# salemmohammed/Distributed-TensorFlow-Guide

Measured on AMD Instinct MI355X. Metric: images/sec (whole node) ResNet-50 sync DP at 1/2/4/8 MI355X; scaling efficiency, higher is better.
Workload: dtype bf16; 1 GPU; model=ResNet-50, global_batch=1024, per_gpu_batch=1024, image_size=224, optimizer=momentum-sgd (fused), parallelism=dp1, allreduce=rccl bf16, 8 MB buckets, overlapped, step_launch=eager

## Files before the change

csrc/bindings/ops.cc:

```cpp
#include <torch/extension.h>
#include <c10/core/DeviceGuard.h>
#include <c10/hip/HIPStream.h>

#include "dtg/kernels.h"

namespace {

using at::Tensor;
using dtg::bf16_t;

hipStream_t cur_stream() { return c10::hip::getCurrentHIPStream().stream(); }

at::Tensor zeros_f32(long long n, const at::Tensor& like) {
  c10::DeviceGuard dg(like.device());
  at::Tensor t = at::empty({n}, like.options().dtype(at::kFloat));
  dtg::fill_zero(t.data_ptr(), n * 4, cur_stream());
  return t;
}

#define CHECK_CUDA(x) TORCH_CHECK((x).is_cuda(), #x " must be a GPU tensor")
#define CHECK_CONTIG(x) TORCH_CHECK((x).is_contiguous(), #x " must be contiguous")
#define CHECK_DT(x, dt) TORCH_CHECK((x).scalar_type() == (dt), #x " must be " #dt)
#define CHECK_IN(x) \
  CHECK_CUDA(x);    \
// ... 707 lines not shown
    CHECK_DT(*bias, at::kFloat);
    TORCH_CHECK(bias->numel() == N, "bias size mismatch");
    bptr = bias->data_ptr<float>();
  }
  void* auxp = nullptr;
  if (aux_mode != 0) {
    TORCH_CHECK(aux_mode >= 1 && aux_mode <= 4, "aux_mode in {0, 1, 2, 3, 4}");
    TORCH_CHECK(aux_mode != 3 || act != 0, "aux_mode 3 stores act'(pre): needs an activation");
    TORCH_CHECK(aux.has_value() && aux->defined(), "aux_mode needs an aux tensor");
    TORCH_CHECK(aux->is_cuda() && aux->scalar_type() == at::kBFloat16 && aux->dim() == 2, "aux must be bf16 2-D");
    TORCH_CHECK(aux->size(0) == M && aux->size(1) == N && aux->stride(0) == out.stride(0) && aux->stride(1) == 1,
                "aux must match out's shape and row stride");
    auxp = aux->data_ptr();
  }
  c10::DeviceGuard dg(A.device());
  if (colsum.has_value() && colsum->defined()) {
    CHECK_IN(*colsum);
    CHECK_DT(*colsum, at::kFloat);
    TORCH_CHECK(colsum->numel() == N, "colsum must hold N floats");
    TORCH_CHECK(a_kc && !b_kc && out.scalar_type() == at::kBFloat16 && alpha == 1.0 && beta == 0.0,
                "colsum epilogue: A [M,K], B [K,N], bf16 out, alpha 1, beta 0");
    TORCH_CHECK(out.stride(0) % 8 == 0 && N % 8 == 0 && ((uintptr_t)out.data_ptr() % 16) == 0 &&
                    (bptr == nullptr || ((uintptr_t)bptr % 16) == 0) && (auxp == nullptr || ((uintptr_t)auxp % 16) == 0),
                "colsum epilogue needs 16-byte aligned rows");
    dtg::gemm_bf16_colsum(cbfp(A), A.stride(0), cbfp(B), B.stride(0), bfp(out), out.stride(0), M, N, K, bptr, (int)act,
                          auxp, (int)aux_mode, colsum->data_ptr<float>(), cur_stream());
    return;
  }
  int sk = split_k > 0 ? (int)split_k : dtg::gemm_pick_split(M, N, K, a_kc ? 1 : 0);
  Tensor ws;
  float* wsp = nullptr;
  if (sk > 1) {
    ws = at::empty({dtg::gemm_workspace_floats(M, N, K, sk)}, A.options().dtype(at::kFloat));
    wsp = ws.data_ptr<float>();
  }
  dtg::gemm_bf16(cbfp(A), A.stride(0), a_kc, cbfp(B), B.stride(0), b_kc, out.data_ptr(), out.stride(0),
                 out.scalar_type() == at::kBFloat16, M, N, K, (float)alpha, (float)beta, bptr, (int)act, sk, wsp,
                 cur_stream(), dtg::GemmBatch(), auxp, (int)aux_mode);
}

void check_nhwc(const Tensor& t, const char* what) {
  CHECK_CUDA(t);
  TORCH_CHECK(t.scalar_type() == at::kBFloat16, what, " must be bf16");
  TORCH_CHECK(t.dim() == 4 && t.is_contiguous(), what, " must be a contiguous [N,H,W,C] tensor");
  TORCH_CHECK(((uintptr_t)t.data_ptr() % 16) == 0, what, " must be 16-byte aligned");
}

bool conv_supported(int64_t C, int64_t K, int64_t R, int64_t S, int64_t stride, int64_t pad, int64_t which) {
  return dtg::conv_supported((int)C, (int)K, (int)R, (int)S, (int)stride, (int)pad, (int)which) != 0;
}

Tensor conv_fwd(Tensor x, Tensor w, int64_t stride, int64_t pad) {
  check_nhwc(x, "x");
  check_nhwc(w, "w");
  const int N = x.size(0), H = x.size(1), W = x.size(2), C = x.size(3);
  const int K = w.size(0), R = w.size(1), S = w.size(2);
  TORCH_CHECK(w.size(3) == C, "weight channels mismatch");
  TORCH_CHECK(dtg::conv_supported(C, K, R, S, stride, pad, 0), "conv shape not supported by the HIP kernel");
  const int P = (H + 2 * pad - R) / stride + 1, Q = (W + 2 * pad - S) / stride + 1;
  TORCH_CHECK(P > 0 && Q > 0, "empty output");
  TORCH_CHECK((long long)N * H * W * C < (1LL << 31) && (long long)N * P * Q * K < (1LL << 31), "tensor too large");
  c10::DeviceGuard dg(x.device());
  auto y = at::empty({N, P, Q, K}, x.options());
  dtg::conv_fwd(cbfp(x), cbfp(w), bfp(y), N, H, W, C, K, R, S, stride, pad, cur_stream());
  return y;
}


Tensor conv_dgrad(Tensor dy, Tensor w, int64_t H, int64_t W, int64_t stride, int64_t pad, c10::optional<Tensor> out,
                  double beta, bool zero_rest) {
  check_nhwc(dy, "dy");
  check_nhwc(w, "w");
  const int N = dy.size(0), P = dy.size(1), Q = dy.size(2), K = dy.size(3);
  const int R = w.size(1), S = w.size(2), C = w.size(3);
  TORCH_CHECK(w.size(0) == K, "weight/dy channel mismatch");
  TORCH_CHECK(dtg::conv_supported(C, K, R, S, stride, pad, 1), "dgrad shape not supported by the HIP kernel");
  TORCH_CHECK((H + 2 * pad - R) / stride + 1 == P && (W + 2 * pad - S) / stride + 1 == Q, "dgrad geometry mismatch");
  c10::DeviceGuard dg(dy.device());
  Tensor dx;
  if (out.has_value()) {
    dx = *out;
    check_nhwc(dx, "out");
    TORCH_CHECK(dx.size(0) == N && dx.size(1) == H && dx.size(2) == W && dx.size(3) == C, "out shape mismatch");
  } else {
    TORCH_CHECK(beta == 0.0, "beta != 0 needs out");
    dx = at::empty({N, H, W, C}, dy.options());
  }
  Tensor wT;
  TORCH_CHECK(zero_rest || (stride == 2 && R == 1 && S == 1 && pad == 0 && beta == 0.0),
              "zero_rest=False is for a stride-2 1x1 dgrad (beta 0)");
  dtg::conv_dgrad(cbfp(dy), cbfp(w), bfp(dx), N, H, W, C, K, R, S, stride, pad, (float)beta, cur_stream(),
                  dtg::BnEpi(), wT.defined() ? cbfp(wT) : nullptr, zero_rest ? 1 : 0);
  return dx;
}

std::tuple<Tensor, Tensor> conv_fwd_c8(Tensor x, Tensor w, int64_t R, int64_t S, int64_t stride, int64_t pad,
                                       bool with_stats, int64_t stride_w) {
  check_nhwc(x, "x");
  CHECK_IN(w);
  CHECK_DT(w, at::kBFloat16);
  const int sw = stride_w > 0 ? (int)stride_w : (int)stride;
  const int N = x.size(0), H = x.size(1), W = x.size(2), K = w.size(0);
  TORCH_CHECK(x.size(3) == 8, "conv_fwd_c8 needs 8 input channels");
  TORCH_CHECK(w.dim() == 2 && w.size(1) == (R * S * 8 + 63) / 64 * 64, "w must be [K, ceil64(R*S*8)]");
  TORCH_CHECK(K % 64 == 0, "K % 64");
  TORCH_CHECK(stride > 0 && sw > 0 && pad >= 0, "bad stride / pad");
  const int P = (H + 2 * pad - R) / stride + 1, Q = (W + 2 * pad - S) / sw + 1;
  TORCH_CHECK(P > 0 && Q > 0 && (long long)N * P * Q * K < (1LL << 31), "bad geometry");
  c10::DeviceGuard dg(x.device());
  auto y = at::empty({N, P, Q, K}, x.options());
  Tensor part;
  dtg::BnEpi bn;
  if (with_stats) {
    part = zeros_f32((long long)dtg::kBnStatSlots * 2 * K, x);
    bn.part = part.data_ptr<float>();
    bn.mode = 1;
  } else {
    part = at::empty({0}, x.options().dtype(at::kFloat));
  }
  dtg::conv_fwd_c8(cbfp(x), cbfp(w), bfp(y), N, H, W, K, (int)R, (int)S, (int)stride, (int)pad, cur_stream(), bn, sw);
  return {y, part};
}

constexpr int kPartRing = 16;
constexpr long long kPartCap = (long long)dtg::kBnStatSlots * 2 * 2048;
Tensor bn_part(const Tensor& like, int64_t C, bool pooled = false) {
  if (!pooled || C > 2048) return zeros_f32((long long)dtg::kBnStatSlots * 2 * C, like);
  static Tensor* ring = new Tensor[64];
  static int next[64] = {0};
  const int dev = like.get_device();
  TORCH_CHECK(dev >= 0 && dev < 64, "device index");
  if (!ring[dev].defined()) ring[dev] = zeros_f32((long long)kPartRing * kPartCap, like);
  const int i = next[dev]++ % kPartRing;
  return ring[dev].narrow(0, i * kPartCap, (long long)dtg::kBnStatSlots * 2 * C);
}

dtg::BnEpi bn_bwd_epi(Tensor& part, const Tensor& x, const Tensor& mean, const Tensor& invstd, const Tensor& gamma,
                      const Tensor& beta, long long M, int C) {
  CHECK_IN(x);
  CHECK_DT(x, at::kBFloat16);
  TORCH_CHECK(x.numel() == M * C, "BN input shape mismatch");
  for (const Tensor* t : {&mean, &invstd, &gamma, &beta}) {
    CHECK_IN(*t);
    CHECK_DT(*t, at::kFloat);
    TORCH_CHECK(t->numel() == C, "per-channel tensor size mismatch");
  }
  dtg::BnEpi bn;
  bn.part = part.data_ptr<float>();
  bn.mode = 2;
  bn.x = cbfp(x);
  bn.mean = mean.data_ptr<float>();
  bn.invstd = invstd.data_ptr<float>();
  bn.gamma = gamma.data_ptr<float>();
  bn.beta = beta.data_ptr<float>();
  return bn;
}

std::tuple<Tensor, Tensor> gemm_bn(Tensor A, Tensor B, int64_t mode, c10::optional<Tensor> x,
                                   c10::optional<Tensor> mean, c10::optional<Tensor> invstd,
                                   c10::optional<Tensor> gamma, c10::optional<Tensor> beta,
                                   c10::optional<Tensor> mask, c10::optional<Tensor> out, bool pooled,
                                   c10::optional<Tensor> x2, c10::optional<Tensor> mean2,
                                   c10::optional<Tensor> invstd2, c10::optional<Tensor> part2,
                                   c10::optional<std::tuple<int64_t, int64_t>> sub2_hw) {
  CHECK_IN(A);
  CHECK_DT(A, at::kBFloat16);
  CHECK_CUDA(B);
  CHECK_DT(B, at::kBFloat16);
  TORCH_CHECK(mode >= 1 && mode <= 3, "mode in {1, 2, 3}");
  TORCH_CHECK(A.dim() == 2 && B.dim() == 2 && B.stride(1) == 1, "2-D operands, contiguous rows");
  const int M = (int)A.size(0), K = (int)A.size(1);
  const int N = (int)(mode == 1 ? B.size(0) : B.size(1));
  TORCH_CHECK((mode == 1 ? B.size(1) : B.size(0)) == K, "gemm_bn K mismatch");
  TORCH_CHECK(K % 8 == 0 && N % 8 == 0 && B.stride(0) % 8 == 0, "K, N and row strides must be multiples of 8");
  TORCH_CHECK(((uintptr_t)A.data_ptr() % 16) == 0 && ((uintptr_t)B.data_ptr() % 16) == 0, "16-byte alignment");
  c10::DeviceGuard dg(A.device());
  Tensor o;
  float bt = 0.f;
  if (out.has_value() && out->defined()) {
    TORCH_CHECK(mode == 3, "accumulating into `out` is mode 3 only");
    o = *out;
    CHECK_IN(o);
    CHECK_DT(o, at::kBFloat16);
    TORCH_CHECK(o.numel() == (long long)M * N, "out shape mismatch");
    bt = 1.f;
  } else {
    o = at::empty({M, N}, A.options());
  }
  auto part = bn_part(A, N, pooled);
  dtg::BnEpi bn;
  if (mode >= 2) {
    TORCH_CHECK(x && mean && invstd && gamma && beta, "modes 2/3 need x, mean, invstd, gamma, beta");
    bn = bn_bwd_epi(part, *x, *mean, *invstd, *gamma, *beta, M, N);
    if (mode == 3) {
      TORCH_CHECK(mask.has_value() && mask->defined(), "mode 3 needs the mask tensor");
      CHECK_IN(*mask);
      bn.mode = 3;
      if (x2.has_value() && x2->defined()) {
        TORCH_CHECK(mean2 && invstd2 && part2, "x2 needs mean2, invstd2 and part2");
        CHECK_IN(*x2);
        CHECK_DT(*x2, at::kBFloat16);
        TORCH_CHECK(x2->numel() == (long long)M * N, "x2 shape mismatch");
        for (const Tensor* t : {&*mean2, &*invstd2}) {
          CHECK_IN(*t);
          CHECK_DT(*t, at::kFloat);
          TORCH_CHECK(t->numel() == N, "per-channel tensor size mismatch");
        }
        CHECK_IN(*part2);
        CHECK_DT(*part2, at::kFloat);
        TORCH_CHECK(part2->numel() == (long long)dtg::kBnStatSlots * 2 * N, "part2 size mismatch");
        bn.x2 = cbfp(*x2);
        bn.mean2 = mean2->data_ptr<float>();
        bn.invstd2 = invstd2->data_ptr<float>();
        bn.part2 = part2->data_ptr<float>();
      }
      if (sub2_hw.has_value()) {
        const auto [sh, sw] = *sub2_hw;
        TORCH_CHECK(bt != 0.f && sh > 0 && sw > 0 && (long long)M % (sh * sw) == 0, "sub2_hw needs out and M = N*H*W");
        dtg::bn_sub2_rows(bn, (int)sh, (int)sw);
      }
      if (mask->scalar_type() == at::kByte) {
        TORCH_CHECK(mask->numel() == (long long)M * (N / 8), "mask bits shape mismatch");
        bn.maskbits = mask->data_ptr<uint8_t>();
      } else {
        CHECK_DT(*mask, at::kBFloat16);
        TORCH_CHECK(mask->numel() == (long long)M * N, "mask shape mismatch");
        bn.mask = cbfp(*mask);
      }
    }
  } else {
    bn.part = part.data_ptr<float>();
    bn.mode = 1;
  }
  dtg::gemm_bf16_bn(cbfp(A), A.stride(0), cbfp(B), B.stride(0), bfp(o), N, M, N, K, bt, bn, cur_stream());
  return {o, part};
}

std::tuple<Tensor, Tensor> conv_fwd_bn(Tensor x, Tensor w, int64_t stride, int64_t pad, bool pooled) {
  check_nhwc(x, "x");
  check_nhwc(w, "w");
  const int N = x.size(0), H = x.size(1), W = x.size(2), C = x.size(3);
  const int K = w.size(0), R = w.size(1), S = w.size(2);
  TORCH_CHECK(w.size(3) == C, "weight channels mismatch");
  TORCH_CHECK(dtg::conv_supported(C, K, R, S, stride, pad, 0), "conv shape not supported by the HIP kernel");
  const int P = (H + 2 * pad - R) / stride + 1, Q = (W + 2 * pad - S) / stride + 1;
  TORCH_CHECK(P > 0 && Q > 0, "empty output");
  TORCH_CHECK((long long)N * H * W * C < (1LL << 31) && (long long)N * P * Q * K < (1LL << 31), "tensor too large");
  c10::DeviceGuard dg(x.device());
  auto y = at::empty({N, P, Q, K}, x.options());
  auto part = bn_part(x, K, pooled);
  dtg::BnEpi bn;
  bn.part = part.data_ptr<float>();
  bn.mode = 1;
  dtg::conv_fwd(cbfp(x), cbfp(w), bfp(y), N, H, W, C, K, R, S, stride, pad, cur_stream(), bn);
  return {y, part};
}

uint8_t* bits_ptr(const c10::optional<Tensor>& bits, long long M, int C) {
  if (!bits.has_value() || !bits->defined()) return nullptr;
  CHECK_IN(*bits);
  TORCH_CHECK(bits->scalar_type() == at::kByte && bits->numel() == M * (C / 8), "bits must be uint8 [M, C/8]");
  return bits->data_ptr<uint8_t>();
}

std::tuple<Tensor, Tensor> conv_dgrad_bn(Tensor dy, Tensor w, int64_t H, int64_t W, int64_t stride, int64_t pad,
                                         Tensor x, Tensor mean, Tensor invstd, Tensor gamma, Tensor beta,
                                         bool pooled, c10::optional<Tensor> bits) {
  check_nhwc(dy, "dy");
  check_nhwc(w, "w");
  const int N = dy.size(0), P = dy.size(1), Q = dy.size(2), K = dy.size(3);
  const int R = w.size(1), S = w.size(2), C = w.size(3);
  TORCH_CHECK(w.size(0) == K, "weight/dy channel mismatch");
  TORCH_CHECK(dtg::conv_supported(C, K, R, S, stride, pad, 1), "dgrad shape not supported by the HIP kernel");
  TORCH_CHECK((H + 2 * pad - R) / stride + 1 == P && (W + 2 * pad - S) / stride + 1 == Q, "dgrad geometry mismatch");
  c10::DeviceGuard dg(dy.device());
  auto dx = at::empty({N, H, W, C}, dy.options());
  auto part = bn_part(dy, C, pooled);
  dtg::BnEpi bn = bn_bwd_epi(part, x, mean, invstd, gamma, beta, (long long)N * H * W, C);
  if (uint8_t* mb = bits_ptr(bits, (long long)N * H * W, C)) {
    bn.mode = 3;
    bn.maskbits = mb;
  }
  Tensor wT;
  TORCH_CHECK(dtg::conv_dgrad(cbfp(dy), cbfp(w), bfp(dx), N, H, W, C, K, R, S, stride, pad, 0.f, cur_stream(), bn,
                              wT.defined() ? cbfp(wT) : nullptr),
              "conv_dgrad_bn: geometry leaves rows unwritten (use conv_dgrad + bn_bwd)");
  return {dx, part};
}

static void check_f32(std::initializer_list<const Tensor*> ts, long long n, const char* what) {
  for (const Tensor* t : ts) {
    CHECK_IN(*t);
    CHECK_DT(*t, at::kFloat);
    TORCH_CHECK(t->numel() == n, what, " size mismatch");
  }
}
static void check_per_channel(std::initializer_list<const Tensor*> ts, int C) {
  check_f32(ts, C, "per-channel tensor");
}
static void check_partials(std::initializer_list<const Tensor*> ts, int C) {
  check_f32(ts, (long long)dtg::kBnStatSlots * 2 * C, "partials");
}

std::tuple<Tensor, Tensor, Tensor> bn_fwd_part(Tensor x, Tensor part, c10::optional<Tensor> res, Tensor gamma,
                                               Tensor beta, Tensor rmean, Tensor rvar, double momentum, double eps,
                                               bool relu, c10::optional<Tensor> bits) {
  CHECK_IN(x);
  CHECK_DT(x, at::kBFloat16);
  TORCH_CHECK(x.dim() == 2, "x must be [M, C]");
  const long long M = x.size(0);
  const int C = (int)x.size(1);
  TORCH_CHECK(C % 8 == 0, "C must be a multiple of 8");
  check_partials({&part}, C);
  check_per_channel({&gamma, &beta, &rmean, &rvar}, C);
  const bool has_res = res.has_value() && res->defined();
  if (has_res) {
    CHECK_IN(*res);
    CHECK_DT(*res, at::kBFloat16);
    TORCH_CHECK(res->sizes() == x.sizes(), "residual shape mismatch");
  }
  c10::DeviceGuard dg(x.device());
  auto y = at::empty_like(x);
  auto fopt = x.options().dtype(at::kFloat);
  auto smean = at::empty({C}, fopt), sinv = at::empty({C}, fopt), ws = at::empty({2LL * C}, fopt);
  dtg::bn_fwd_from_part(cbfp(x), has_res ? cbfp(*res) : nullptr, bfp(y), gamma.data_ptr<float>(),
                        beta.data_ptr<float>(), rmean.data_ptr<float>(), rvar.data_ptr<float>(),
                        smean.data_ptr<float>(), sinv.data_ptr<float>(), part.data_ptr<float>(), ws.data_ptr<float>(),
                        M, C, (float)momentum, (float)eps, relu, cur_stream(), bits_ptr(bits, M, C));
  return {y, smean, sinv};
}

std::tuple<Tensor, Tensor, Tensor, Tensor, Tensor> bn_fwd2_part(Tensor x, Tensor part, Tensor gamma, Tensor beta,
                                                                Tensor rmean, Tensor rvar, Tensor r, Tensor part2,
                                                                Tensor gamma2, Tensor beta2, Tensor rmean2,
                                                                Tensor rvar2, double momentum, double eps,
                                                                c10::optional<Tensor> bits) {
  CHECK_IN(x);
  CHECK_IN(r);
  CHECK_DT(x, at::kBFloat16);
  CHECK_DT(r, at::kBFloat16);
  TORCH_CHECK(x.dim() == 2 && r.sizes() == x.sizes(), "x/r must be [M, C]");
  const long long M = x.size(0);
  const int C = (int)x.size(1);
  TORCH_CHECK(C % 8 == 0, "C must be a multiple of 8");
  check_partials({&part, &part2}, C);
  check_per_channel({&gamma, &beta, &rmean, &rvar, &gamma2, &beta2, &rmean2, &rvar2}, C);
  c10::DeviceGuard dg(x.device());
  auto y = at::empty_like(x);
  auto fopt = x.options().dtype(at::kFloat);
  auto m1 = at::empty({C}, fopt), i1 = at::empty({C}, fopt), m2 = at::empty({C}, fopt), i2 = at::empty({C}, fopt);
  auto ws = at::empty({4LL * C}, fopt);
  dtg::bn_fwd2_from_part(cbfp(x), cbfp(r), bfp(y), part.data_ptr<float>(), part2.data_ptr<float>(),
                         gamma.data_ptr<float>(), beta.data_ptr<float>(), rmean.data_ptr<float>(),
                         rvar.data_ptr<float>(), m1.data_ptr<float>(), i1.data_ptr<float>(), gamma2.data_ptr<float>(),
                         beta2.data_ptr<float>(), rmean2.data_ptr<float>(), rvar2.data_ptr<float>(),
                         m2.data_ptr<float>(), i2.data_ptr<float>(), ws.data_ptr<float>(), M, C, (float)momentum,
                         (float)eps, cur_stream(), bits_ptr(bits, M, C));
  return {y, m1, i1, m2, i2};
}

static void check_wgrad_fuse(const Tensor& x, const c10::optional<Tensor>& wact, const c10::optional<Tensor>& wgrad) {
  TORCH_CHECK(wact.has_value() && wgrad.has_value() && wact->defined() && wgrad->defined(), "wact needs wgrad");
  CHECK_CUDA(*wact);
  CHECK_DT(*wact, at::kBFloat16);
  CHECK_IN(*wgrad);
  TORCH_CHECK(wgrad->scalar_type() == at::kFloat || wgrad->scalar_type() == at::kBFloat16, "wgrad fp32/bf16");
  const long long M = x.size(0);
  const int C = (int)x.size(1), CI = (int)wact->size(1);
  TORCH_CHECK(wact->dim() == 2 && wact->size(0) == M && wact->stride(1) == 1 && wact->stride(0) % 8 == 0 &&
                  ((uintptr_t)wact->data_ptr() % 16) == 0,
              "wact must be [M, CI] with 16-byte aligned rows");
  TORCH_CHECK(wgrad->numel() == (long long)C * CI, "wgrad must be [C, CI]");
  TORCH_CHECK(dtg::bn_dx_wgrad_ok(M, C, CI), "fused dx + wgrad: unsupported shape (see bn_dx_wgrad_ok)");
}

struct DgradFuse {
  c10::optional<Tensor> w, y, mean, invstd, bits, part;
  bool full = false;
  bool on() const { return w.has_value() && w->defined(); }
};

static dtg::DxDgrad check_dgrad_fuse(const Tensor& x, const c10::optional<Tensor>& wact, const DgradFuse& f,
                                     const Tensor& dpo) {
  TORCH_CHECK(wact.has_value() && wact->defined(), "the fused dgrad rides on the fused weight gradient (wact)");
  for (const c10::optional<Tensor>* t : {&f.y, &f.mean, &f.invstd, &f.bits, &f.part})
    TORCH_CHECK(t->has_value() && (*t)->defined(), "dgw needs dgy, dgmean, dginv, dgbits and dgpart");
  const long long M = x.size(0);
  const int C = (int)x.size(1), CI = (int)wact->size(1);
  TORCH_CHECK(f.full || dtg::bn_dx_dgrad_ok(M, C, CI), "fused dx + dgrad: unsupported shape (see bn_dx_dgrad_ok)");
  TORCH_CHECK(!f.full || dtg::bn_dx_dgrad_full_ok(M, C, CI),
              "fused dx + dgrad: unsupported shape (see bn_dx_dgrad_full_ok)");
  CHECK_CUDA(*f.w);
  CHECK_DT(*f.w, at::kBFloat16);
  TORCH_CHECK(f.w->dim() == 2 && f.w->size(0) == C && f.w->size(1) == CI && f.w->stride(1) == 1 &&
                  f.w->stride(0) % 8 == 0 && ((uintptr_t)f.w->data_ptr() % 16) == 0,
              "dgw must be [C, CI] with 16-byte aligned rows");
  CHECK_IN(*f.y);
  CHECK_DT(*f.y, at::kBFloat16);
  TORCH_CHECK(f.y->dim() == 2 && f.y->size(0) == M && f.y->size(1) == CI && ((uintptr_t)f.y->data_ptr() % 16) == 0,
              "dgy must be [M, CI], 16-byte aligned");
  check_per_channel({&*f.mean, &*f.invstd}, CI);
  check_partials({&*f.part}, CI);
  dtg::DxDgrad d;
  d.w = cbfp(*f.w);
  d.ldw = f.w->stride(0);
  d.y = cbfp(*f.y);
  d.mean = f.mean->data_ptr<float>();
  d.invstd = f.invstd->data_ptr<float>();
  d.bits = bits_ptr(f.bits, M, CI);
  d.dp = bfp(dpo);
  d.part = f.part->data_ptr<float>();
  return d;
}

struct DxFuseSide {
  const Tensor &x, &part, &gamma, &smean, &sinv, &dgamma, &dbeta;
  const Tensor& dx;
  const c10::optional<Tensor> &wact, &wgrad;
};

static Tensor bn_dx_wgrad_fused(const Tensor& dp, const DxFuseSide& a, const DxFuseSide* b, const Tensor& ws, int accum,
                                const DgradFuse& dgf) {
  const long long M = a.x.size(0);
  const int C = (int)a.x.size(1);
  check_wgrad_fuse(a.x, a.wact, a.wgrad);
  const int CI = (int)a.wact->size(1);
  const bool w2 = b && b->wact.has_value() && b->wact->defined();
  if (w2) {
    check_wgrad_fuse(b->x, b->wact, b->wgrad);
    TORCH_CHECK(C == 256 && CI == 64 && b->wact->size(1) == CI && b->wgrad->scalar_type() == a.wgrad->scalar_type(),
                "wact2: 256 x 64 only, wgrad2 of wgrad's dtype");
  }
  Tensor dpo;
  dtg::DxDgrad dgd;
  if (dgf.on()) {
    TORCH_CHECK(!b || w2, "dgw in the dual form needs wact2");
    dpo = at::empty({M, (long long)CI}, a.x.options());
    dgd = check_dgrad_fuse(a.x, a.wact, dgf, dpo);
  }
  const long long ns = (long long)dtg::bn_dx_wgrad_slabs(C, CI, w2, dgf.on()) * C * CI;
  auto slabs = at::empty({w2 ? 2 * ns : ns}, a.x.options().dtype(at::kFloat));
  auto side = [&](const DxFuseSide& s, int k) {
    dtg::DxSide d;
    d.x = cbfp(s.x);
    float* coef = ws.data_ptr<float>() + k * 3LL * C;
    dtg::bn_bwd_coef_from_part(s.part.data_ptr<float>(), s.gamma.data_ptr<float>(), s.smean.data_ptr<float>(),
                               s.sinv.data_ptr<float>(), coef, s.dgamma.data_ptr<float>(), s.dbeta.data_ptr<float>(),
                               M, C, accum, cur_stream());
    d.coef = coef;
    d.dx = s.dx.defined() ? bfp(s.dx) : nullptr;
    if (s.wact.has_value() && s.wact->defined()) {
      d.act = cbfp(*s.wact);
      d.ldact = s.wact->stride(0);
      d.wgrad = s.wgrad->data_ptr();
      d.slabs = slabs.data_ptr<float>() + k * ns;
    }
    return d;
  };
  const dtg::DxSide da = side(a, 0), db = b ? side(*b, 1) : dtg::DxSide{};
  dtg::bn_dx_wgrad(cbfp(dp), da, b ? &db : nullptr, M, C, CI, a.wgrad->scalar_type() == at::kBFloat16, cur_stream(),
                   dgf.on() ? &dgd : nullptr);
  return dpo;
}

pybind11::tuple bn_bwd2_part(Tensor dp, Tensor x, Tensor part, Tensor gamma, Tensor smean, Tensor sinv,
                             Tensor dgamma, Tensor dbeta, Tensor x2, Tensor part2, Tensor gamma2,
                             Tensor smean2, Tensor sinv2, Tensor dgamma2, Tensor dbeta2,
                             c10::optional<Tensor> wact, c10::optional<Tensor> wgrad,
                             c10::optional<Tensor> wact2, c10::optional<Tensor> wgrad2,
                             c10::optional<Tensor> dgw, c10::optional<Tensor> dgy, c10::optional<Tensor> dgmean,
                             c10::optional<Tensor> dginv, c10::optional<Tensor> dgbits,
                             c10::optional<Tensor> dgpart, bool dgfull) {
  const DgradFuse dgf{dgw, dgy, dgmean, dginv, dgbits, dgpart, dgfull};
  TORCH_CHECK(!(dgfull && dgf.on()), "dgfull: the full-width fused dgrad has no dual form (bn_bwd_part only)");
  for (const Tensor* t : {&dp, &x, &x2}) {
    CHECK_IN(*t);
    CHECK_DT(*t, at::kBFloat16);
  }
  TORCH_CHECK(x.dim() == 2 && dp.numel() == x.numel() && x2.sizes() == x.sizes(), "dp/x/x2 must be [M, C]");
  const long long M = x.size(0);
  const int C = (int)x.size(1);
  TORCH_CHECK(C % 8 == 0, "C must be a multiple of 8");
  check_partials({&part, &part2}, C);
  check_per_channel({&gamma, &smean, &sinv, &dgamma, &dbeta, &gamma2, &smean2, &sinv2, &dgamma2, &dbeta2}, C);
  c10::DeviceGuard dg(x.device());
  TORCH_CHECK(!dgf.on() || (wact.has_value() && wact->defined()), "dgw needs wact");
  Tensor dx, dx2 = at::empty_like(x);
  if (!dgf.on()) dx = at::empty_like(x);
  auto ws = at::empty({6LL * C}, x.options().dtype(at::kFloat));
  if (wact.has_value() && wact->defined()) {
    const DxFuseSide a{x, part, gamma, smean, sinv, dgamma, dbeta, dx, wact, wgrad};
    const DxFuseSide b{x2, part2, gamma2, smean2, sinv2, dgamma2, dbeta2, dx2, wact2, wgrad2};
    const Tensor dpo = bn_dx_wgrad_fused(dp, a, &b, ws, 1, dgf);
    if (dgf.on()) return pybind11::make_tuple(pybind11::none(), dx2, dpo, *dgf.part);
    return pybind11::make_tuple(dx, dx2);
  }
  dtg::bn_bwd2_from_part(cbfp(dp), cbfp(x), cbfp(x2), part.data_ptr<float>(), part2.data_ptr<float>(),
                         gamma.data_ptr<float>(), smean.data_ptr<float>(), sinv.data_ptr<float>(),
                         gamma2.data_ptr<float>(), smean2.data_ptr<float>(), sinv2.data_ptr<float>(), bfp(dx),
                         bfp(dx2), dgamma.data_ptr<float>(), dbeta.data_ptr<float>(), dgamma2.data_ptr<float>(),
                         dbeta2.data_ptr<float>(), ws.data_ptr<float>(), M, C, 1, cur_stream());
  return pybind11::make_tuple(dx, dx2);
}

pybind11::tuple bn_bwd_part(Tensor dp, Tensor x, Tensor part, Tensor gamma, Tensor smean, Tensor sinv, bool want_dres,
                            c10::optional<Tensor> dgamma_acc, c10::optional<Tensor> dbeta_acc,
                            c10::optional<Tensor> wact, c10::optional<Tensor> wgrad, c10::optional<Tensor> dgw,
                            c10::optional<Tensor> dgy, c10::optional<Tensor> dgmean, c10::optional<Tensor> dginv,
                            c10::optional<Tensor> dgbits, c10::optional<Tensor> dgpart, bool dgfull) {
  const DgradFuse dgf{dgw, dgy, dgmean, dginv, dgbits, dgpart, dgfull};
  CHECK_IN(dp);
  CHECK_IN(x);
  CHECK_DT(dp, at::kBFloat16);
  CHECK_DT(x, at::kBFloat16);
  TORCH_CHECK(x.dim() == 2 && dp.numel() == x.numel(), "dp/x must be [M, C]");
  const long long M = x.size(0);
  const int C = (int)x.size(1);
  TORCH_CHECK(C % 8 == 0, "C must be a multiple of 8");
  check_partials({&part}, C);
  check_per_channel({&gamma, &smean, &sinv}, C);
  c10::DeviceGuard dg(x.device());
  TORCH_CHECK(!dgf.on() || (wact.has_value() && wact->defined()), "dgw needs wact");
  Tensor dx;
  if (!dgf.on()) dx = at::empty_like(x);
  c10::optional<Tensor> dres;
  if (want_dres) dres = at::empty_like(x);
  auto fopt = x.options().dtype(at::kFloat);
  const bool acc = dgamma_acc.has_value() && dgamma_acc->defined() && dbeta_acc.has_value() && dbeta_acc->defined();
  Tensor dgamma, dbeta;
  if (acc) {
    dgamma = *dgamma_acc;
    dbeta = *dbeta_acc;
    check_per_channel({&dgamma, &dbeta}, C);
  } else {
    dgamma = at::empty({C}, fopt);
    dbeta = at::empty({C}, fopt);
  }
  auto ws = at::empty({3LL * C}, fopt);
  if (wact.has_value() && wact->defined()) {
    TORCH_CHECK(!want_dres, "fused dx + wgrad: no dres");
    const Tensor dpo =
        bn_dx_wgrad_fused(dp, {x, part, gamma, smean, sinv, dgamma, dbeta, dx, wact, wgrad}, nullptr, ws, acc, dgf);
    if (dgf.on()) return pybind11::make_tuple(pybind11::none(), dres, dgamma, dbeta, dpo, *dgf.part);
    return pybind11::make_tuple(dx, dres, dgamma, dbeta);
  }
  dtg::bn_bwd_from_part(cbfp(dp), cbfp(x), gamma.data_ptr<float>(), smean.data_ptr<float>(), sinv.data_ptr<float>(),
                        part.data_ptr<float>(), bfp(dx), want_dres ? bfp(*dres) : nullptr, dgamma.data_ptr<float>(),
                        dbeta.data_ptr<float>(), ws.data_ptr<float>(), M, C, acc, cur_stream());
  return pybind11::make_tuple(dx, dres, dgamma, dbeta);
}

void conv_wgrad(Tensor dy, Tensor x, Tensor dw, double beta, int64_t stride, int64_t pad, int64_t stride_w,
                int64_t target_wgs, int64_t sched) {
  check_nhwc(dy, "dy");
  check_nhwc(x, "x");
  CHECK_CUDA(dw);
  TORCH_CHECK(dw.dim() == 4 && dw.is_contiguous(), "dw must be contiguous [K,R,S,C]");
  TORCH_CHECK(dw.scalar_type() == at::kFloat || dw.scalar_type() == at::kBFloat16, "dw fp32/bf16");
  const int N = x.size(0), H = x.size(1), W = x.size(2), C = x.size(3);
  const int K = dw.size(0), R = dw.size(1), S = dw.size(2);
  TORCH_CHECK(dw.size(3) == C && dy.size(3) == K && dy.size(0) == N, "wgrad shape mismatch");
  TORCH_CHECK(dtg::conv_supported(C, K, R, S, stride, pad, 2), "wgrad shape not supported by the HIP kernel");
  const int sw = stride_w > 0 ? (int)stride_w : (int)stride;
  const int P = (H + 2 * pad - R) / stride + 1, Q = (W + 2 * pad - S) / sw + 1;
  TORCH_CHECK(dy.size(1) == P && dy.size(2) == Q, "wgrad geometry mismatch");
  c10::DeviceGuard dg(x.device());
  const int split = dtg::conv_wgrad_split(N, H, W, C, K, R, S, stride, pad, sw, (int)target_wgs);
  auto ws = at::empty({(long long)split * K * R * S * C}, x.options().dtype(at::kFloat));
  dtg::conv_wgrad(cbfp(dy), cbfp(x), dw.data_ptr(), dw.scalar_type() == at::kBFloat16, (float)beta,
                  ws.data_ptr<float>(), split, N, H, W, C, K, R, S, stride, pad, cur_stream(), sw, (int)sched);
}

}

void register_transformer_ops(pybind11::module_& m);
void register_pool_ops(pybind11::module_& m);
void register_data_ops(pybind11::module_& m);
void register_eval_ops(pybind11::module_& m);
void register_mlm_ops(pybind11::module_& m);

PYBIND11_MODULE(TORCH_EXTENSION_NAME, m) {
  m.def("conv_supported", &conv_supported);
  m.def("conv_fwd", &conv_fwd);
  m.def("conv_dgrad", &conv_dgrad, pybind11::arg("dy"), pybind11::arg("w"), pybind11::arg("H"), pybind11::arg("W"),
        pybind11::arg("stride"), pybind11::arg("pad"), pybind11::arg("out") = pybind11::none(),
        pybind11::arg("beta") = 0.0, pybind11::arg("zero_rest") = true);
  m.def("conv_wgrad", &conv_wgrad, pybind11::arg("dy"), pybind11::arg("x"), pybind11::arg("dw"),
        pybind11::arg("beta"), pybind11::arg("stride"), pybind11::arg("pad"), pybind11::arg("stride_w") = 0,
        pybind11::arg("target_wgs") = 0, pybind11::arg("sched") = 0);
  m.def("gemm_bn", &gemm_bn, pybind11::arg("A"), pybind11::arg("B"), pybind11::arg("mode"),
        pybind11::arg("x") = pybind11::none(), pybind11::arg("mean") = pybind11::none(),
        pybind11::arg("invstd") = pybind11::none(), pybind11::arg("gamma") = pybind11::none(),
        pybind11::arg("beta") = pybind11::none(), pybind11::arg("mask") = pybind11::none(),
        pybind11::arg("out") = pybind11::none(), pybind11::arg("pooled") = false,
        pybind11::arg("x2") = pybind11::none(), pybind11::arg("mean2") = pybind11::none(),
        pybind11::arg("invstd2") = pybind11::none(), pybind11::arg("part2") = pybind11::none(),
        pybind11::arg("sub2_hw") = pybind11::none());
  m.def("bn_part_alloc", [](Tensor like, int64_t C, bool pooled) { return bn_part(like, C, pooled); },
        pybind11::arg("like"), pybind11::arg("C"), pybind11::arg("pooled") = false);
  m.def("bn_bwd2_part", &bn_bwd2_part, pybind11::arg("dp"), pybind11::arg("x"), pybind11::arg("part"),
        pybind11::arg("gamma"), pybind11::arg("smean"), pybind11::arg("sinv"), pybind11::arg("dgamma"),
        pybind11::arg("dbeta"), pybind11::arg("x2"), pybind11::arg("part2"), pybind11::arg("gamma2"),
        pybind11::arg("smean2"), pybind11::arg("sinv2"), pybind11::arg("dgamma2"), pybind11::arg("dbeta2"),
        pybind11::arg("wact") = pybind11::none(), pybind11::arg("wgrad") = pybind11::none(),
        pybind11::arg("wact2") = pybind11::none(), pybind11::arg("wgrad2") = pybind11::none(),
        pybind11::arg("dgw") = pybind11::none(), pybind11::arg("dgy") = pybind11::none(),
        pybind11::arg("dgmean") = pybind11::none(), pybind11::arg("dginv") = pybind11::none(),
        pybind11::arg("dgbits") = pybind11::none(), pybind11::arg("dgpart") = pybind11::none(),
        pybind11::arg("dgfull") = false);
  m.def("bn_dx_wgrad_ok", [](int64_t M, int64_t C, int64_t CI) { return dtg::bn_dx_wgrad_ok(M, (int)C, (int)CI); });
  m.def("bn_dx_dgrad_ok", [](int64_t M, int64_t C, int64_t CI) { return dtg::bn_dx_dgrad_ok(M, (int)C, (int)CI); });
  m.def("bn_dx_dgrad_full_ok",
        [](int64_t M, int64_t C, int64_t CI) { return dtg::bn_dx_dgrad_full_ok(M, (int)C, (int)CI); });
  m.def("bn_dx_wgrad_slabs",
        [](int64_t C, int64_t CI, int64_t w2, bool dg) { return dtg::bn_dx_wgrad_slabs((int)C, (int)CI, (int)w2, dg); },
        pybind11::arg("C"), pybind11::arg("CI"), pybind11::arg("w2") = 0, pybind11::arg("dg") = false);
  m.def("conv_fwd_bn", &conv_fwd_bn, pybind11::arg("x"), pybind11::arg("w"), pybind11::arg("stride"),
        pybind11::arg("pad"), pybind11::arg("pooled") = false);
  m.def("conv_dgrad_bn", &conv_dgrad_bn, pybind11::arg("dy"), pybind11::arg("w"), pybind11::arg("H"),
        pybind11::arg("W"), pybind11::arg("stride"), pybind11::arg("pad"), pybind11::arg("x"), pybind11::arg("mean"),
        pybind11::arg("invstd"), pybind11::arg("gamma"), pybind11::arg("beta"), pybind11::arg("pooled") = false,
        pybind11::arg("bits") = pybind11::none());
  m.def("bn_fwd2_part", &bn_fwd2_part, pybind11::arg("x"), pybind11::arg("part"), pybind11::arg("gamma"),
        pybind11::arg("beta"), pybind11::arg("rmean"), pybind11::arg("rvar"), pybind11::arg("r"), pybind11::arg("part2"),
        pybind11::arg("gamma2"), pybind11::arg("beta2"), pybind11::arg("rmean2"), pybind11::arg("rvar2"),
        pybind11::arg("momentum"), pybind11::arg("eps"), pybind11::arg("bits") = pybind11::none());
  m.def("conv_fwd_c8", &conv_fwd_c8, pybind11::arg("x"), pybind11::arg("w"), pybind11::arg("R"), pybind11::arg("S"),
        pybind11::arg("stride"), pybind11::arg("pad"), pybind11::arg("with_stats") = false,
        pybind11::arg("stride_w") = 0);
  m.def("bn_fwd_part", &bn_fwd_part, pybind11::arg("x"), pybind11::arg("part"), pybind11::arg("res"),
        pybind11::arg("gamma"), pybind11::arg("beta"), pybind11::arg("rmean"), pybind11::arg("rvar"),
        pybind11::arg("momentum"), pybind11::arg("eps"), pybind11::arg("relu"), pybind11::arg("bits") = pybind11::none());
  m.def("bn_bwd_part", &bn_bwd_part, pybind11::arg("dp"), pybind11::arg("x"), pybind11::arg("part"),
        pybind11::arg("gamma"), pybind11::arg("smean"), pybind11::arg("sinv"), pybind11::arg("want_dres"),
        pybind11::arg("dgamma_acc") = pybind11::none(), pybind11::arg("dbeta_acc") = pybind11::none(),
        pybind11::arg("wact") = pybind11::none(), pybind11::arg("wgrad") = pybind11::none(),
        pybind11::arg("dgw") = pybind11::none(), pybind11::arg("dgy") = pybind11::none(),
        pybind11::arg("dgmean") = pybind11::none(), pybind11::arg("dginv") = pybind11::none(),
        pybind11::arg("dgbits") = pybind11::none(), pybind11::arg("dgpart") = pybind11::none(),
        pybind11::arg("dgfull") = false);
  m.doc() = "dtg gfx950 HIP kernels";
  {
    namespace py = pybind11;
    m.def("sgd_apply", &sgd_apply, py::arg("w"), py::arg("mirror"), py::arg("g"), py::arg("hyper"), py::arg("wd"),
          py::arg("gscale"), py::arg("zero_grad"), py::arg("clip") = py::none());
    m.def("momentum_apply", &momentum_apply, py::arg("w"), py::arg("mirror"), py::arg("g"), py::arg("mom"),
          py::arg("hyper"), py::arg("mu"), py::arg("wd"), py::arg("nesterov"), py::arg("gscale"), py::arg("zero_grad"),
          py::arg("clip") = py::none());
    m.def("adagrad_apply", &adagrad_apply, py::arg("w"), py::arg("mirror"), py::arg("g"), py::arg("acc"),
          py::arg("hyper"), py::arg("eps"), py::arg("gscale"), py::arg("zero_grad"), py::arg("clip") = py::none());
    m.def("adam_apply", &adam_apply, py::arg("w"), py::arg("mirror"), py::arg("g"), py::arg("m"), py::arg("v"),
          py::arg("hyper"), py::arg("b1"), py::arg("b2"), py::arg("eps"), py::arg("wd"), py::arg("gscale"),
          py::arg("zero_grad"), py::arg("clip") = py::none());
  }
  m.attr("LW_CHUNK") = (int)dtg::kLwChunk;
  m.attr("LW_SERIAL") = (int)dtg::kLwSerial;
  m.attr("LW_TREE_DEPTH") = (int)dtg::kLwTreeDepth;
  m.def("lw_chunk_table", &lw_chunk_table);
  m.def("seg_sqnorm", &seg_sqnorm);
  m.def("lamb_moments", &lamb_moments);
  m.def("lamb_apply", &lamb_apply);
  m.def("lars_apply", &lars_apply);
  m.def("seg_finalize", &seg_finalize);
  m.def("axpby", &axpby);
  m.def("sgd_sum_apply", &sgd_sum_apply);
  m.def("momentum_sum_apply", &momentum_sum_apply);
  m.def("adagrad_sum_apply", &adagrad_sum_apply);
  m.def("adam_sum_apply", &adam_sum_apply);
  m.def("grad_sum", &grad_sum);
  m.def("grad_fold", &grad_fold);
  m.def("grad_unfold", &grad_unfold);
  m.def("state_chunk_table", &state_chunk_table);
  m.def("state_pack", &state_pack);
  m.def("state_unpack", &state_unpack);
  m.def("comm_spin", [](double seconds, int64_t wgs, int64_t lds_bytes) {
    dtg::comm_spin(seconds, (int)wgs, (int)lds_bytes, cur_stream());
  }, pybind11::arg("seconds"), pybind11::arg("wgs") = 32, pybind11::arg("lds_bytes") = 0);
  m.def("comm_emu", [](double seconds, int64_t wgs, int64_t mode, c10::optional<Tensor> scratch, int64_t base,
                       int64_t traffic_bytes, c10::optional<Tensor> bucket, double factor) {
    long long sbytes = 0, n = 0;
    int bf = 0;
    const Tensor* dev_t = nullptr;
    if (scratch.has_value() && scratch->defined()) {
      CHECK_IN(*scratch);
      TORCH_CHECK(((uintptr_t)scratch->data_ptr() % 16) == 0, "scratch: 16-B aligned");
      sbytes = scratch->numel() * scratch->element_size();
      dev_t = &*scratch;
    }
    if (bucket.has_value() && bucket->defined()) {
      CHECK_IN(*bucket);
      TORCH_CHECK(bucket->scalar_type() == at::kFloat || bucket->scalar_type() == at::kBFloat16, "bucket fp32/bf16");
      n = bucket->numel();
      bf = bucket->scalar_type() == at::kBFloat16;
      dev_t = &*bucket;
    }
    TORCH_CHECK(!(mode & 2) || sbytes > 0, "traffic mode needs scratch");
    TORCH_CHECK(!(mode & 4) || n > 0 || !(bucket.has_value() && bucket->defined()), "data mode needs the bucket");
    c10::optional<c10::DeviceGuard> dg;
    if (dev_t) dg.emplace(dev_t->device());
    return dtg::comm_emu(seconds, (int)wgs, (int)mode, sbytes ? scratch->data_ptr() : nullptr, sbytes, base,
                         traffic_bytes, n ? bucket->data_ptr() : nullptr, n, bf, (float)factor, cur_stream());
  }, pybind11::arg("seconds"), pybind11::arg("wgs") = 32, pybind11::arg("mode") = 0,
        pybind11::arg("scratch") = pybind11::none(), pybind11::arg("base") = 0, pybind11::arg("traffic_bytes") = 0,
        pybind11::arg("bucket") = pybind11::none(), pybind11::arg("factor") = 1.0);
  m.def("stem_stream_set", [](int64_t on) { dtg::stem_stream_set((int)on); });
  m.def("gemm_expand_k256_set", [](int64_t on) { dtg::gemm_expand_k256_set((int)on); });
  m.def("stem_pool_rows_set", [](int64_t on) { dtg::stem_pool_rows_set((int)on); });
  m.def("gemm_expand_s2_set", [](int64_t on) { dtg::gemm_expand_s2_set((int)on); });
  m.def("conv_halo_fwd_set", [](int64_t on) { dtg::conv3x3_halo_fwd_set((int)on); });
  m.def("conv_halo_dgrad_set", [](int64_t on) { dtg::conv3x3_halo_dgrad_set((int)on); });
  m.def("conv_halo_wgrad_set", [](int64_t on) { dtg::conv3x3_halo_wgrad_set((int)on); });
  m.def("conv_lin_wgrad_set", [](int64_t on) { dtg::conv3x3_lin_wgrad_set((int)on); });
  m.def("hyper_tick", [](Tensor hyper) {
    check_hyper(hyper);
    c10::DeviceGuard dg(hyper.device());
    dtg::hyper_tick(hyper.data_ptr<float>(), cur_stream());
  });
  m.def("stem_pack_weights", [](Tensor w) {
    CHECK_CUDA(w);
    CHECK_DT(w, at::kBFloat16);
    TORCH_CHECK(w.dim() == 4 && w.is_contiguous(at::MemoryFormat::ChannelsLast) && w.size(1) <= 4,
                "w: channels_last [K, C<=4, R, S]");
    const int K = w.size(0), C = w.size(1), R = w.size(2), S = w.size(3), S2 = (S + 1) / 2;
    const int KP = (R * S2 * 8 + 63) / 64 * 64;
    c10::DeviceGuard dg(w.device());
    auto wp = at::empty({K, KP}, w.options().memory_format(at::MemoryFormat::Contiguous));
    dtg::stem_pack_weights(cbfp(w), bfp(wp), K, C, R, S, S2, KP, cur_stream());
    return wp;
  });
  m.def("stem_dw_add", [](Tensor src, Tensor grad, bool pair) {
    CHECK_IN(src);
    CHECK_DT(src, at::kFloat);
    CHECK_CUDA(grad);
    TORCH_CHECK(grad.dim() == 4 && grad.is_contiguous(at::MemoryFormat::ChannelsLast), "grad: channels_last [K,C,R,S]");
    TORCH_CHECK(grad.scalar_type() == at::kFloat || grad.scalar_type() == at::kBFloat16, "grad fp32/bf16");
    const int K = grad.size(0), C = grad.size(1), R = grad.size(2), S = grad.size(3);
    TORCH_CHECK(src.dim() == 4 && src.size(0) == K && src.size(1) == R && src.size(3) == 8 && C <= 4 &&
                    src.size(2) == (pair ? (S + 1) / 2 : S), "stem dw source shape");
    c10::DeviceGuard dg(grad.device());
    dtg::stem_dw_add(src.data_ptr<float>(), grad.data_ptr(), grad.scalar_type() == at::kBFloat16, K, R, S, C,
                     (int)src.size(2), pair ? 1 : 0, cur_stream());
  });
  m.def("stream_probe", [](int64_t kind, Tensor a, c10::optional<Tensor> b, c10::optional<Tensor> o, Tensor sink,
                           int64_t wgs, int64_t unroll, bool nt) {
    CHECK_IN(a);
    CHECK_IN(sink);
    TORCH_CHECK(sink.scalar_type() == at::kInt && sink.numel() >= wgs, "sink: int32 with >= wgs elements");
    const long long bytes = a.numel() * a.element_size();
    TORCH_CHECK(bytes % 16 == 0 && ((uintptr_t)a.data_ptr() % 16) == 0, "a: 16-B multiple, 16-B aligned");
    for (const auto* t : {&b, &o})
      if (t->has_value() && (*t)->defined()) {
        CHECK_IN(**t);
        TORCH_CHECK((*t)->numel() * (*t)->element_size() == bytes && ((uintptr_t)(*t)->data_ptr() % 16) == 0,
                    "b / o: the byte size of a, 16-B aligned");
      }
    TORCH_CHECK(kind >= 0 && kind <= 3, "kind 0..3");
    TORCH_CHECK(kind == 0 || (o.has_value() && o->defined()), "kinds 1-3 write o");
    TORCH_CHECK(kind != 3 || (b.has_value() && b->defined()), "kind 3 reads b");
    TORCH_CHECK(wgs >= 1 && wgs <= 65536, "wgs");
    c10::DeviceGuard dg(a.device());
    dtg::stream_probe((int)kind, a.data_ptr(), opt_ptr<void>(b), opt_ptr<void>(o), bytes / 16,
                      reinterpret_cast<unsigned*>(sink.data_ptr()), (int)wgs, (int)unroll, nt ? 1 : 0, cur_stream());
  }, pybind11::arg("kind"), pybind11::arg("a"), pybind11::arg("b") = pybind11::none(),
        pybind11::arg("o") = pybind11::none(), pybind11::arg("sink"), pybind11::arg("wgs") = 1024,
        pybind11::arg("unroll") = 4, pybind11::arg("nt") = false);
  m.def("launch_probe", [](int64_t grid, int64_t lds_bytes) {
    dtg::launch_probe((int)grid, (int)lds_bytes, cur_stream());
  });
  m.def("f32_to_bf16", &f32_to_bf16);
  m.def("bn_fwd_train", &bn_fwd_train);
  m.def("bn_fwd_infer", &bn_fwd_infer);
  m.def("bn_bwd", &bn_bwd, pybind11::arg("dy"), pybind11::arg("y"), pybind11::arg("x"), pybind11::arg("gamma"),
        pybind11::arg("smean"), pybind11::arg("sinv"), pybind11::arg("relu"), pybind11::arg("want_dres"),
        pybind11::arg("dgamma_acc") = pybind11::none(), pybind11::arg("dbeta_acc") = pybind11::none());
  m.def("softmax_xent", &softmax_xent);
  m.def("gemm_bn_force_cfg", [](int64_t c) { dtg::gemm_bn_force_cfg((int)c); });
  m.def("conv_force_tile", [](int64_t which, int64_t c) { dtg::conv_force_tile((int)which, (int)c); });
  m.def("conv_set_stages", [](int64_t which, int64_t s) { dtg::conv_set_stages((int)which, (int)s); });
  m.def("softmax_xent_bwd", &softmax_xent_bwd);
  m.def("gemm_pick_split", [](int64_t M, int64_t N, int64_t K, bool a_kc, int64_t target_wgs) {
    return dtg::gemm_pick_split((int)M, (int)N, (int)K, a_kc ? 1 : 0, (int)target_wgs);
  }, pybind11::arg("M"), pybind11::arg("N"), pybind11::arg("K"), pybind11::arg("a_kc") = false,
        pybind11::arg("target_wgs") = 0);
  m.def("gemm", &gemm, pybind11::arg("A"), pybind11::arg("a_kc"), pybind11::arg("B"), pybind11::arg("b_kc"),
        pybind11::arg("out"), pybind11::arg("alpha") = 1.0, pybind11::arg("beta") = 0.0,
        pybind11::arg("bias") = pybind11::none(), pybind11::arg("act") = 0, pybind11::arg("split_k") = 0,
        pybind11::arg("aux") = pybind11::none(), pybind11::arg("aux_mode") = 0,
        pybind11::arg("colsum") = pybind11::none());
  register_transformer_ops(m);
  register_pool_ops(m);
  register_data_ops(m);
  register_eval_ops(m);
  register_mlm_ops(m);
}
```

csrc/include/dtg/kernels.h:

```cpp
#pragma once
#include <hip/hip_runtime.h>
#include <stdint.h>

namespace dtg {
typedef unsigned short bf16_t;

void sgd_apply(float* w, bf16_t* mirror, void* grad, int grad_bf16, long long n, const float* hyper, float wd,
               float gscale, int zero_grad, hipStream_t st, const float* clip = nullptr);
void momentum_apply(float* w, bf16_t* mirror, void* grad, int grad_bf16, float* mom, long long n,
                    const float* hyper, float mu, float wd, int nesterov, float gscale, int zero_grad,
                    hipStream_t st, const float* clip = nullptr);
void adagrad_apply(float* w, bf16_t* mirror, void* grad, int grad_bf16, float* acc, long long n,
                   const float* hyper, float eps, float gscale, int zero_grad, hipStream_t st,
                   const float* clip = nullptr);
void adam_apply(float* w, bf16_t* mirror, void* grad, int grad_bf16, float* m, float* v, long long n,
                const float* hyper, float b1, float b2, float eps, float wd, float gscale, int zero_grad,
                hipStream_t st, const float* clip = nullptr);
void axpby(float* acc, const void* g, int g_bf16, long long n, float alpha, float beta, hipStream_t st);
void f32_to_bf16(const float* x, bf16_t* y, long long n, hipStream_t st);
void hyper_tick(float* hyper, hipStream_t st);
struct GradSrcs {
  const void* p[8] = {nullptr, nullptr, nullptr, nullptr, nullptr, nullptr, nullptr, nullptr};
};
void sgd_sum_apply(float* w, bf16_t* mirror, const float* acc, const GradSrcs& src, int k, int src_bf16, long long n,
                   const float* hyper, float wd, float gscale, hipStream_t st);
void momentum_sum_apply(float* w, bf16_t* mirror, const float* acc, const GradSrcs& src, int k, int src_bf16,
                        float* mom, long long n, const float* hyper, float mu, float wd, int nesterov, float gscale,
                        hipStream_t st);
void adagrad_sum_apply(float* w, bf16_t* mirror, const float* acc, const GradSrcs& src, int k, int src_bf16,
                       float* slot, long long n, const float* hyper, float eps, float gscale, hipStream_t st);
void adam_sum_apply(float* w, bf16_t* mirror, const float* acc, const GradSrcs& src, int k, int src_bf16, float* m,
                    float* v, long long n, const float* hyper, float b1, float b2, float eps, float wd, float gscale,
                    hipStream_t st);
void grad_sum(float* acc, const GradSrcs& src, int k, int src_bf16, long long n, int first, float scale,
              hipStream_t st);
void grad_fold(float* acc, void* g, int g_bf16, long long n, int first, hipStream_t st);
void grad_unfold(void* g, int g_bf16, const float* acc, long long lo, long long hi, hipStream_t st);
constexpr int kMaxStateSrcs = 4;
constexpr int kStateChunk = 2048;
struct StatePtrs {
  float* p[4] = {nullptr, nullptr, nullptr, nullptr};
};
void state_pack(const StatePtrs& src, int k, float* image, long long n, const long long* rows, const int* chunks,
                int n_chunks, hipStream_t st);
void state_unpack(const StatePtrs& dst, int k, const float* image, long long n, const long long* rows,
                  const int* chunks, int n_chunks, hipStream_t st);
constexpr int kLwChunk = 2048;
constexpr int kLwSerial = 8;
constexpr int kLwTreeDepth = 8;
constexpr int kMaxLwGroups = 4;
enum { kLwNone = 0, kLwLars = 1, kLwLamb = 2 };
struct LwGroups {
  int row_end[4] = {0x7fffffff, 0x7fffffff, 0x7fffffff, 0x7fffffff};
  int adapt[4] = {0, 0, 0, 0};
  float wd[4] = {0.f, 0.f, 0.f, 0.f};
};
void seg_sqnorm(const float* w, const void* grad, int grad_bf16, const long long* rows, const int* chunks, int c_lo,
                int n_chunks, float* partials, int C, hipStream_t st);
void lamb_moments(const float* w, void* grad, int grad_bf16, float* m, float* v, const long long* rows,
                  const int* chunks, int c_lo, int n_chunks, float* partials, int C, const float* hyper, double b1,
                  double b2, float eps, float wd, float gscale, const float* cfac, int zero_grad, hipStream_t st);
void lamb_apply(float* w, bf16_t* mirror, const float* m, const float* v, const long long* rows, const int* chunks,
                int c_lo, int n_chunks, const float* hyper, double b1, double b2, float eps, float wd,
                const float* ratio, hipStream_t st);
void lars_apply(float* w, bf16_t* mirror, void* grad, int grad_bf16, float* mom, const long long* rows,
                const int* chunks, int c_lo, int n_chunks, const float* hyper, float mu, float wd, float gscale,
                const float* cfac, const float* ratio, int zero_grad, hipStream_t st);
void seg_finalize(const float* partials, int C, const long long* rows, int P, const LwGroups& grp, int rule,
                  float clip_norm, float gscale, float eta, float eps, float* norms, float* ratio, float* cfac,
                  hipStream_t st);
void mul_bf16(const bf16_t* a, const bf16_t* b, bf16_t* out, long long n, hipStream_t st);
void mask_additive(const void* mask, int is_f32, float* out, long long n, hipStream_t st);
void fill_zero(void* p, long long bytes, hipStream_t st);

void comm_spin(double seconds, int wgs, int lds_bytes, hipStream_t st);
long long comm_emu(double seconds, int wgs, int mode, void* scratch, long long scratch_bytes, long long base,
                   long long traffic_bytes, void* buf, long long n, int buf_bf16, float factor, hipStream_t st);
void launch_probe(int grid, int lds_bytes, hipStream_t st);
void stream_probe(int kind, const void* a, const void* b, void* o, long long n16, unsigned* sink, int wgs, int unroll,
                  int nt, hipStream_t st);

constexpr int kBnStatSlots = 32;
struct BnEpi {
  float* part = nullptr;
  int mode = 0;
  const bf16_t* x = nullptr;
  const float* mean = nullptr;
  const float* invstd = nullptr;
  const float* gamma = nullptr;
  const float* beta = nullptr;
  const bf16_t* mask = nullptr;
  const uint8_t* maskbits = nullptr;
  const bf16_t* x2 = nullptr;
  const float* mean2 = nullptr;
  const float* invstd2 = nullptr;
  float* part2 = nullptr;
  int old_sub2 = 0;
  uint32_t old_hw = 1, old_w = 1, hw_m = 0, hw_l = 0, w_m = 0, w_l = 0;
};

inline void bn_sub2_rows(BnEpi& bn, int H, int W) {
  auto magic = [](uint32_t d, uint32_t& m, uint32_t& l) {
    l = 0;
    while ((1u << l) < d) ++l;
    m = (uint32_t)((((uint64_t)1 << 32) * (((uint64_t)1 << l) - d)) / d + 1);
  };
  bn.old_sub2 = 1;
  bn.old_hw = (uint32_t)(H * W);
  bn.old_w = (uint32_t)W;
  magic(bn.old_hw, bn.hw_m, bn.hw_l);
  magic(bn.old_w, bn.w_m, bn.w_l);
}

long long bn_workspace_floats(long long M, int C);
void bn_fwd_from_part(const bf16_t* x, const bf16_t* res, bf16_t* y, const float* gamma, const float* beta,
                      float* rmean, float* rvar, float* smean, float* sinv, const float* part, float* ws, long long M,
                      int C, float momentum, float eps, int relu, hipStream_t st, uint8_t* bits = nullptr);
void bn_fwd2_from_part(const bf16_t* x, const bf16_t* r, bf16_t* y, const float* part, const float* part2,
                       const float* gamma, const float* beta, float* rmean, float* rvar, float* smean, float* sinv,
                       const float* gamma2, const float* beta2, float* rmean2, float* rvar2, float* smean2,
                       float* sinv2, float* ws, long long M, int C, float momentum, float eps, hipStream_t st,
                       uint8_t* bits = nullptr);
void bn_bwd2_from_part(const bf16_t* dp, const bf16_t* x, const bf16_t* x2, const float* part, const float* part2,
                       const float* gamma, const float* smean, const float* sinv, const float* gamma2,
                       const float* smean2, const float* sinv2, bf16_t* dx, bf16_t* dx2, float* dgamma, float* dbeta,
                       float* dgamma2, float* dbeta2, float* ws, long long M, int C, int accum, hipStream_t st);
void bn_bwd_coef_from_part(const float* part, const float* gamma, const float* smean, const float* sinv, float* coef,
                           float* dgamma, float* dbeta, long long M, int C, int accum, hipStream_t st);
void bn_dx_from_coef(const bf16_t* dp, const bf16_t* x, const float* coef, bf16_t* dx, bf16_t* dres, long long M, int C,
                     hipStream_t st);
bool bn_dx_wgrad_ok(long long M, int C, int CI);
struct DxDgrad {
  const bf16_t* w = nullptr;
  long long ldw = 0;
  const bf16_t* y = nullptr;
  const float* mean = nullptr;
  const float* invstd = nullptr;
  const uint8_t* bits = nullptr;
  bf16_t* dp = nullptr;
  float* part = nullptr;
};
bool bn_dx_dgrad_ok(long long M, int C, int CI);
bool bn_dx_dgrad_full_ok(long long M, int C, int CI);
int bn_dx_wgrad_slabs(int C, int CI, int w2 = 0, int dg = 0);
struct DxSide {
  const bf16_t* x = nullptr;
  const float* coef = nullptr;
  bf16_t* dx = nullptr;
  const bf16_t* act = nullptr;
  long long ldact = 0;
  void* wgrad = nullptr;
  float* slabs = nullptr;
};
void bn_dx_wgrad(const bf16_t* dp, const DxSide& main, const DxSide* second, long long M, int C, int CI,
                 int wgrad_bf16, hipStream_t st, const DxDgrad* dg = nullptr);
void bn_bwd_from_part(const bf16_t* dp, const bf16_t* x, const float* gamma, const float* smean, const float* sinv,
                      const float* part, bf16_t* dx, bf16_t* dres, float* dgamma, float* dbeta, float* ws, long long M,
                      int C, int accum, hipStream_t st);
void bn_fwd_train(const bf16_t* x, const bf16_t* res, bf16_t* y, const float* gamma, const float* beta,
                  float* rmean, float* rvar, float* smean, float* sinv, float* ws, long long M, int C,
                  float momentum, float eps, int relu, hipStream_t st);
void bn_fwd_infer(const bf16_t* x, const bf16_t* res, bf16_t* y, const float* gamma, const float* beta,
                  const float* rmean, const float* rvar, float* ws, long long M, int C, float eps, int relu,
                  hipStream_t st);
void bn_bwd(const bf16_t* dy, const bf16_t* y, const bf16_t* x, const float* gamma, const float* smean,
            const float* sinv, bf16_t* dx, bf16_t* dres, float* dgamma, float* dbeta, float* ws, long long M, int C,
            int relu, int accum, hipStream_t st);

void softmax_xent(const void* x, int x_bf16, const long long* label, long long B, int V, float scale, float* loss,
                  void* dx, float* lse, hipStream_t st);
void softmax_xent_bwd(const void* x, int x_bf16, const long long* label, const float* lse, long long B, int V,
                      float scale, const float* g, void* dx, hipStream_t st);

void xent_rank(const void* x, int x_bf16, const long long* label, long long B, int V, float* loss, int* rank,
               hipStream_t st);
void metric_accumulate(const float* loss, const int* rank, long long B, int V, const int* ks, int nk, double* acc,
                       hipStream_t st);

struct GemmBatch {
  int count = 1, nh = 1;
  long long sa_b = 0, sa_h = 0, sb_b = 0, sb_h = 0, sc_b = 0, sc_h = 0;
};
void gemm_bn_force_cfg(int cfg);
void conv_force_tile(int which, int code);
long long gemm_workspace_floats(int M, int N, int K, int split_k);
int gemm_pick_split(int M, int N, int K, int a_kc = 0, int target_wgs = 0);
void gemm_bf16(const bf16_t* A, long long lda, int a_kc, const bf16_t* B, long long ldb, int b_kc, void* C,
               long long ldc, int c_bf16, int M, int N, int K, float alpha, float beta, const float* bias, int act,
               int split_k, float* ws, hipStream_t st, const GemmBatch& batch = GemmBatch(), void* aux = nullptr,
               int aux_mode = 0);
void gemm_bf16_bn(const bf16_t* A, long long lda, const bf16_t* B, long long ldb, bf16_t* C, long long ldc, int M,
                  int N, int K, float beta, const BnEpi& bn, hipStream_t st);
void gemm_bf16_colsum(const bf16_t* A, long long lda, const bf16_t* B, long long ldb, bf16_t* C, long long ldc, int M,
                      int N, int K, const float* bias, int act, void* aux, int aux_mode, float* colsum, hipStream_t st);

int ln_max_hidden();
void ln_fwd(const bf16_t* h, const bf16_t* res, const float* gamma, const float* beta, bf16_t* y, bf16_t* s_out,
            float* mean, float* rstd, int T, int H, float eps, float p_in, uint32_t seed_in, float p_out,
            uint32_t seed_out, hipStream_t st);
int ln_bwd_blocks(int T);
void ln_bwd(const bf16_t* dy, const bf16_t* s, const float* gamma, const float* mean, const float* rstd,
            bf16_t* ds_out, bf16_t* dh_out, float* dgamma, float* dbeta, float* dbias, float* ws, int T, int H,
            float p_in, uint32_t seed_in, float p_out, uint32_t seed_out, hipStream_t st);
int attn_max_keys();
void attn_softmax_fwd(const float* sc, const float* mask, bf16_t* P, bf16_t* Pd, int rows, int rows_per_b, int Sk,
                      float p, uint32_t seed, hipStream_t st);
void attn_softmax_bwd(const bf16_t* P, const bf16_t* Pd, const float* dPd, bf16_t* dS, int rows, int Sk, float scale,
                      hipStream_t st);
int colsum_splits(int T, int N);
void colsum(const bf16_t* x, long long ld, int T, int N, const long long* sel, int nsel, void* out, int out_bf16,
            int accumulate, float* ws, int splits, hipStream_t st);
void emb_fwd(const long long* ids, const long long* tt, const bf16_t* word, const bf16_t* pos, const bf16_t* type,
             bf16_t* s, int T, int S, int H, hipStream_t st);
void emb_word_bwd(const bf16_t* ds, const long long* sorted, const long long* perm, bf16_t* gW, int T, int H,
                  hipStream_t st);
void emb_pos_bwd(const bf16_t* ds, bf16_t* gP, int T, int S, int H, hipStream_t st);

void gather_rows(const bf16_t* src, const long long* pos, bf16_t* out, int R, int P, int S, int H, hipStream_t st);
void scatter_rows_add(bf16_t* dst, const long long* pos, const bf16_t* src, int R, int P, int S, int H,
                      hipStream_t st);
void nsp_loss_fwd(const bf16_t* pooled, const bf16_t* wn, const float* bn, const long long* labels, const float* extra,
                  float* probs, float* out, int B, int H, hipStream_t st);
void nsp_loss_bwd(const bf16_t* pooled, const bf16_t* wn, const float* probs, const long long* labels, const float* gout,
                  bf16_t* dpre, bf16_t* gwn, float* gbn, int B, int H, hipStream_t st);
void row_sum(const float* x, float* out, long long n, float scale, hipStream_t st);
void emb_word_bwd_owned(const bf16_t* ds, const long long* ids, bf16_t* gW, int T, int H, int V, hipStream_t st);

int attn_fused_supported(int S, int dh, int backward);
void attn_fwd(const bf16_t* qkv, const float* mask, bf16_t* out, float* lse, int B, int S, int nh, float p,
              uint32_t seed, hipStream_t st);
void attn_bwd(const bf16_t* qkv, const bf16_t* o, const bf16_t* dout, const float* lse, const float* mask,
              bf16_t* dqkv, int B, int S, int nh, float p, uint32_t seed, float* dbias, hipStream_t st);

void maxpool_fwd(const bf16_t* x, bf16_t* y, uint8_t* idx, int N, int H, int W, int C, int k, int s, int pad, int P,
                 int Q, hipStream_t st);
void maxpool_bwd(const bf16_t* dy, const uint8_t* idx, bf16_t* dx, int N, int H, int W, int C, int k, int s, int pad,
                 int P, int Q, hipStream_t st);
void avgpool_fwd(const bf16_t* x, bf16_t* y, int N, int HW, int C, hipStream_t st);
void avgpool_bwd(const bf16_t* dy, bf16_t* dx, int N, int HW, int C, hipStream_t st);

void stem_bn_pool_fwd(const bf16_t* y, const float* part, const float* gamma, const float* beta, float* rmean,
                      float* rvar, float* smean, float* sinv, float* coef, bf16_t* out, uint8_t* idx, int N, int H,
                      int W, int C, int k, int s, int pad, int P, int Q, float momentum, float eps, hipStream_t st,
                      bf16_t* yam = nullptr);
long long stem_bwd_workspace_floats(long long M, int C);
bool stem_pooled_stats_ok(int C);
void stem_pack_weights(const bf16_t* w, bf16_t* wp, int K, int C, int R, int S, int S2, int KP, hipStream_t st);
void stem_dw_add(const float* src, void* grad, int grad_bf16, int K, int R, int S, int C, int S2, int pair,
                 hipStream_t st);
void stem_pack_pairs(const bf16_t* x, bf16_t* xp, int N, int H, int W, int C, int pad, int Hp, int Wp,
                     hipStream_t st);
void stem_bn_pool_bwd(const bf16_t* dout, const uint8_t* idx, const bf16_t* y, const float* gamma, const float* beta,
                      const float* smean, const float* sinv, bf16_t* dy, float* dgamma, float* dbeta, int accum,
                      float* ws, int N, int H, int W, int C, int k, int s, int pad, int P, int Q, hipStream_t st,
                      const bf16_t* yam = nullptr);

void im2col(const bf16_t* x, bf16_t* cols, int N, int H, int W, int C, int R, int S, int stride, int pad, int Kp,
            hipStream_t st);
void col2im(const bf16_t* dcols, bf16_t* dx, int N, int H, int W, int C, int R, int S, int stride, int pad, int Kp,
            hipStream_t st);

int conv_supported(int C, int K, int R, int S, int stride, int pad, int which);
int conv3x3_halo_bn_ok(int C, int K, int H, int W);
bool conv3x3_halo_bn_fwd(const bf16_t* x, const bf16_t* w, bf16_t* y, int N, int H, int W, float* part, hipStream_t st);
void conv3x3_halo_fwd_set(int on);
bool conv3x3_halo_bn_dgrad(const bf16_t* dy, const bf16_t* w, bf16_t* dp, int N, int H, int W, const BnEpi& bn,
                           hipStream_t st);
void conv3x3_halo_dgrad_set(int on);
int conv3x3_halo_wgrad_split(int N, int H, int W, int C, int K, int R, int S, int stride, int pad, int stride_w);
void conv3x3_halo_wgrad(const bf16_t* dy, const bf16_t* x, float* ws, int grid, int N, int H, hipStream_t st);
void conv3x3_halo_wgrad_set(int on);
int conv3x3_lin_wgrad_split(int N, int H, int W, int C, int K, int R, int S, int stride, int pad, int stride_w);
void conv3x3_lin_wgrad(const bf16_t* dy, const bf16_t* x, float* ws, int split, int N, int H, int W, int C, int K,
                       hipStream_t st);
void conv3x3_lin_wgrad_set(int on);
void conv_fwd(const bf16_t* x, const bf16_t* w, bf16_t* y, int N, int H, int W, int C, int K, int R, int S,
              int stride, int pad, hipStream_t st, const BnEpi& bn = BnEpi());
int conv_dgrad(const bf16_t* dy, const bf16_t* w, bf16_t* dx, int N, int H, int W, int C, int K, int R, int S,
               int stride, int pad, float beta, hipStream_t st, const BnEpi& bn = BnEpi(),
               const bf16_t* wT = nullptr, int zero_rest = 1);
void stem_stream_set(int on);
void stem_pool_rows_set(int on);
void gemm_expand_k256_set(int on);
void gemm_expand_s2_set(int on);
bool conv1x1_s2_expand_bn(const bf16_t* x, int Nb, int H, int W, int Cin, const bf16_t* w, bf16_t* y, int Kout,
                          float* part, hipStream_t st);
void conv_fwd_c8(const bf16_t* x, const bf16_t* w, bf16_t* y, int N, int H, int W, int K, int R, int S, int stride,
                 int pad, hipStream_t st, const BnEpi& bn = BnEpi(), int stride_w = 0);
void conv_set_stages(int which, int stages);
int conv_wgrad_split(int N, int H, int W, int C, int K, int R, int S, int stride, int pad, int stride_w = 0,
                     int target_wgs = 0);
void conv_wgrad(const bf16_t* dy, const bf16_t* x, void* dw, int dw_bf16, float beta, float* ws, int split, int N,
                int H, int W, int C, int K, int R, int S, int stride, int pad, hipStream_t st, int stride_w = 0,
                int sched = 0);

}
```

csrc/kernels/batchnorm.hip:

```cpp
#include <stdlib.h>
#include "dtg/common.h"
#include "dtg/kernels.h"
#include "dtg/bn_finalize.cuh"

namespace dtg {

long long bn_workspace_floats(long long M, int C) {
  BnGeom g = bn_geom(M, C);
  return (long long)g.nchunk * 2 * C + 4LL * C;
}

template <int TPR>
__global__ void __launch_bounds__(kBlk) bn_stats_kernel(const bf16_t* __restrict__ x, long long M, int C,
                                                        long long rpc, float* __restrict__ part) {
  constexpr int RPP = kBlk / TPR, CW = TPR * 8;
  __shared__ float sh[2][RPP][CW + 4];
  const int tx = threadIdx.x % TPR, ty = threadIdx.x / TPR;
  const int c0 = blockIdx.y * CW + tx * 8;
  const long long m0 = (long long)blockIdx.x * rpc;
  const long long m1 = m0 + rpc < M ? m0 + rpc : M;
  float s[8] = {0, 0, 0, 0, 0, 0, 0, 0}, q[8] = {0, 0, 0, 0, 0, 0, 0, 0};
  if (c0 < C) {
    long long m = m0 + ty;
    for (; m + RPP < m1; m += 2 * RPP) {
      float a[8], b[8];
      load8_bf16(x + m * C + c0, a);
      load8_bf16(x + (m + RPP) * C + c0, b);
#pragma unroll
      for (int k = 0; k < 8; ++k) { s[k] += a[k] + b[k]; q[k] += a[k] * a[k] + b[k] * b[k]; }
    }
    if (m < m1) {
      float a[8];
      load8_bf16(x + m * C + c0, a);
#pragma unroll
      for (int k = 0; k < 8; ++k) { s[k] += a[k]; q[k] += a[k] * a[k]; }
    }
  }
#pragma unroll
  for (int k = 0; k < 8; ++k) { sh[0][ty][tx * 8 + k] = s[k]; sh[1][ty][tx * 8 + k] = q[k]; }
  __syncthreads();
  for (int c = threadIdx.x; c < CW; c += kBlk) {
    float ts = 0.f, tq = 0.f;
#pragma unroll 4
    for (int r = 0; r < RPP; ++r) { ts += sh[0][r][c]; tq += sh[1][r][c]; }
    const int cc = blockIdx.y * CW + c;
    if (cc < C) {
      part[((long long)blockIdx.x * 2 + 0) * C + cc] = ts;
      part[((long long)blockIdx.x * 2 + 1) * C + cc] = tq;
    }
  }
}

__device__ __forceinline__ uint8_t pos_bits8(const float (&v)[8]) {
  uint32_t b = 0;
#pragma unroll
  for (int k = 0; k < 8; ++k) b |= (v[k] > 0.f ? 1u : 0u) << k;
  return (uint8_t)b;
}

__device__ __forceinline__ void store_bits(uint8_t* bits, long long off, const float (&v)[8], int tx, int C) {
  const uint32_t b = pos_bits8(v);
  if ((C & 31) == 0) {
    uint32_t w = b << (8 * (tx & 3));
    w |= __shfl_xor(w, 1, 64);
    w |= __shfl_xor(w, 2, 64);
    if ((tx & 3) == 0) *reinterpret_cast<uint32_t*>(bits + (off >> 3)) = w;
  } else {
    bits[off >> 3] = (uint8_t)b;
  }
}

template <int TPR, bool RES, bool RELU, int RU = 4>
__global__ void __launch_bounds__(kBlk) bn_apply_kernel(const bf16_t* __restrict__ x, const bf16_t* __restrict__ res,
                                                        bf16_t* __restrict__ y, const float* __restrict__ coef,
                                                        long long M, int C, long long rpc,
                                                        uint8_t* __restrict__ bits = nullptr) {
  constexpr int RPP = kBlk / TPR, CW = TPR * 8;
  const int tx = threadIdx.x % TPR, ty = threadIdx.x / TPR;
  const int c0 = blockIdx.y * CW + tx * 8;
  if (c0 >= C) return;
  float sc[8], sf[8];
  load8_f32(coef + c0, sc);
  load8_f32(coef + C + c0, sf);
  const long long m0 = (long long)blockIdx.x * rpc;
  const long long m1 = m0 + rpc < M ? m0 + rpc : M;
  auto finish = [&](float (&a)[8], const float (&r)[8], long long off) {
#pragma unroll
    for (int k = 0; k < 8; ++k) {
      float v = a[k] * sc[k] + sf[k];
      if constexpr (RES) v += r[k];
      if constexpr (RELU) v = fmaxf(v, 0.f);
      a[k] = v;
    }
    store8_bf16(y + off, a);
    if (bits) store_bits(bits, off, a, tx, C);
  };
  long long m = m0 + ty;
  for (; m + (RU - 1) * RPP < m1; m += RU * RPP) {
    float a[RU][8], r[RU][8];
#pragma unroll
    for (int u = 0; u < RU; ++u) {
      load8_bf16(x + (m + u * RPP) * C + c0, a[u]);
      if constexpr (RES) load8_bf16(res + (m + u * RPP) * C + c0, r[u]);
    }
#pragma unroll
    for (int u = 0; u < RU; ++u) finish(a[u], r[u], (m + u * RPP) * C + c0);
  }
  for (; m < m1; m += RPP) {
    const long long o0 = m * C + c0;
    float a0[8], r0[8];
    load8_bf16(x + o0, a0);
    if constexpr (RES) load8_bf16(res + o0, r0);
    finish(a0, r0, o0);
  }
}

template <int TPR, int RU = 4>
__global__ void __launch_bounds__(kBlk) bn_apply2_kernel(const bf16_t* __restrict__ x, const bf16_t* __restrict__ r,
                                                         bf16_t* __restrict__ y, const float* __restrict__ coef,
                                                         const float* __restrict__ coef2, long long M, int C,
                                                         long long rpc, uint8_t* __restrict__ bits) {
  constexpr int RPP = kBlk / TPR, CW = TPR * 8;
  const int tx = threadIdx.x % TPR, ty = threadIdx.x / TPR;
  const int c0 = blockIdx.y * CW + tx * 8;
  if (c0 >= C) return;
  float sc[8], sf[8], sc2[8], sf2[8];
  load8_f32(coef + c0, sc);
  load8_f32(coef + C + c0, sf);
  load8_f32(coef2 + c0, sc2);
  load8_f32(coef2 + C + c0, sf2);
#pragma unroll
  for (int k = 0; k < 8; ++k) sf[k] += sf2[k];
  const long long m0 = (long long)blockIdx.x * rpc;
  const long long m1 = m0 + rpc < M ? m0 + rpc : M;
  auto finish = [&](float (&a)[8], const float (&b)[8], long long o) {
#pragma unroll
    for (int k = 0; k < 8; ++k) a[k] = fmaxf(fmaf(a[k], sc[k], fmaf(b[k], sc2[k], sf[k])), 0.f);
    store8_bf16(y + o, a);
    if (bits) store_bits(bits, o, a, tx, C);
  };
  long long m = m0 + ty;
  for (; m + (RU - 1) * RPP < m1; m += RU * RPP) {
    float a[RU][8], b[RU][8];
#pragma unroll
    for (int u = 0; u < RU; ++u) {
      load8_bf16(x + (m + u * RPP) * C + c0, a[u]);
      load8_bf16(r + (m + u * RPP) * C + c0, b[u]);
    }
#pragma unroll
    for (int u = 0; u < RU; ++u) finish(a[u], b[u], (m + u * RPP) * C + c0);
  }
  for (; m < m1; m += RPP) {
    const long long o0 = m * C + c0;
    float a0[8], b0[8];
    load8_bf16(x + o0, a0);
    load8_bf16(r + o0, b0);
    finish(a0, b0, o0);
  }
}

template <int TPR, bool RELU>
__global__ void __launch_bounds__(kBlk) bn_bwd_reduce_kernel(const bf16_t* __restrict__ dy,
                                                             const bf16_t* __restrict__ y,
                                                             const bf16_t* __restrict__ x,
                                                             const float* __restrict__ smean,
                                                             const float* __restrict__ sinv, long long M, int C,
                                                             long long rpc, float* __restrict__ part) {
  constexpr int RPP = kBlk / TPR, CW = TPR * 8;
  __shared__ float sh[2][RPP][CW + 4];
  const int tx = threadIdx.x % TPR, ty = threadIdx.x / TPR;
  const int c0 = blockIdx.y * CW + tx * 8;
  float s[8] = {0, 0, 0, 0, 0, 0, 0, 0}, q[8] = {0, 0, 0, 0, 0, 0, 0, 0};
  if (c0 < C) {
    float mu[8], is[8];
    load8_f32(smean + c0, mu);
    load8_f32(sinv + c0, is);
    const long long m0 = (long long)blockIdx.x * rpc;
    const long long m1 = m0 + rpc < M ? m0 + rpc : M;
    auto acc = [&](float (&g)[8], const float (&xv)[8], const float (&yv)[8]) {
      if constexpr (RELU) {
#pragma unroll
        for (int k = 0; k < 8; ++k) g[k] = yv[k] > 0.f ? g[k] : 0.f;
      }
#pragma unroll
      for (int k = 0; k < 8; ++k) { s[k] += g[k]; q[k] += g[k] * (xv[k] - mu[k]) * is[k]; }
    };
    long long m = m0 + ty;
    for (; m + RPP < m1; m += 2 * RPP) {
      const long long o0 = m * C + c0, o1 = (m + RPP) * C + c0;
      float g0[8], g1[8], x0[8], x1[8], y0[8], y1[8];
      load8_bf16(dy + o0, g0);
      load8_bf16(dy + o1, g1);
      load8_bf16(x + o0, x0);
      load8_bf16(x + o1, x1);
      if constexpr (RELU) {
        load8_bf16(y + o0, y0);
        load8_bf16(y + o1, y1);
      }
      acc(g0, x0, y0);
      acc(g1, x1, y1);
    }
    if (m < m1) {
      const long long o0 = m * C + c0;
      float g0[8], x0[8], y0[8];
      load8_bf16(dy + o0, g0);
      load8_bf16(x + o0, x0);
      if constexpr (RELU) load8_bf16(y + o0, y0);
      acc(g0, x0, y0);
    }
  }
#pragma unroll
  for (int k = 0; k < 8; ++k) { sh[0][ty][tx * 8 + k] = s[k]; sh[1][ty][tx * 8 + k] = q[k]; }
  __syncthreads();
  for (int c = threadIdx.x; c < CW; c += kBlk) {
    float ts = 0.f, tq = 0.f;
#pragma unroll 4
    for (int r = 0; r < RPP; ++r) { ts += sh[0][r][c]; tq += sh[1][r][c]; }
    const int cc = blockIdx.y * CW + c;
    if (cc < C) {
      part[((long long)blockIdx.x * 2 + 0) * C + cc] = ts;
      part[((long long)blockIdx.x * 2 + 1) * C + cc] = tq;
    }
  }
}

template <int TPR, bool RELU, bool DRES, bool NT = true, int RU = 4>
__global__ void __launch_bounds__(kBlk) bn_bwd_dx_kernel(const bf16_t* __restrict__ dy, const bf16_t* __restrict__ y,
                                                         const bf16_t* __restrict__ x, const float* __restrict__ coef,
                                                         bf16_t* __restrict__ dx, bf16_t* __restrict__ dres,
                                                         long long M, int C, long long rpc) {
  constexpr int RPP = kBlk / TPR, CW = TPR * 8;
  const int tx = threadIdx.x % TPR, ty = threadIdx.x / TPR;
  const int c0 = blockIdx.y * CW + tx * 8;
  if (c0 >= C) return;
  float a[8], bx[8], cc[8];
  load8_f32(coef + c0, a);
  load8_f32(coef + C + c0, bx);
  load8_f32(coef + 2 * C + c0, cc);
  const long long m0 = (long long)blockIdx.x * rpc;
  const long long m1 = m0 + rpc < M ? m0 + rpc : M;
  auto finish = [&](float (&g)[8], const float (&xv)[8], const float (&yv)[8], long long off) {
    if constexpr (RELU) {
#pragma unroll
      for (int k = 0; k < 8; ++k) g[k] = yv[k] > 0.f ? g[k] : 0.f;
    }
    if constexpr (DRES) store8_bf16(dres + off, g);
    float o[8];
#pragma unroll
    for (int k = 0; k < 8; ++k) o[k] = a[k] * g[k] + bx[k] * xv[k] + cc[k];
    store8_bf16(dx + off, o);
  };
  auto ld = [&](const bf16_t* p, float (&v)[8]) {
    if constexpr (NT) load8_bf16_nt(p, v);
    else load8_bf16(p, v);
  };
  long long m = m0 + ty;
  for (; m + (RU - 1) * RPP < m1; m += RU * RPP) {
    float g[RU][8], xv[RU][8], yv[RU][8];
#pragma unroll
    for (int u = 0; u < RU; ++u) {
      const long long o = (m + u * RPP) * C + c0;
      ld(dy + o, g[u]);
      ld(x + o, xv[u]);
      if constexpr (RELU) load8_bf16(y + o, yv[u]);
    }
#pragma unroll
    for (int u = 0; u < RU; ++u) finish(g[u], xv[u], yv[u], (m + u * RPP) * C + c0);
  }
  for (; m < m1; m += RPP) {
    const long long o0 = m * C + c0;
    float g0[8], x0[8], y0[8];
    ld(dy + o0, g0);
    ld(x + o0, x0);
    if constexpr (RELU) load8_bf16(y + o0, y0);
    finish(g0, x0, y0, o0);
  }
}

#define DTG_RU_SWITCH(...) \
  { constexpr int RU = 2; __VA_ARGS__; }

static void bn_apply_launch(const BnGeom& g, const bf16_t* x, const bf16_t* res, bf16_t* y, const float* coef,
                            long long M, int C, int relu, hipStream_t st, uint8_t* bits = nullptr) {
  const long long rpa = elementwise_rpc(g, M);
  dim3 ga((unsigned)((M + rpa - 1) / rpa), g.gy);
  DTG_TPR_SWITCH(g.tpr, DTG_RU_SWITCH({
    if (res) {
      if (relu) { bn_apply_kernel<T, true, true, RU><<<ga, kBlk, 0, st>>>(x, res, y, coef, M, C, rpa, bits); DTG_LAUNCH_CHECK(); }
      else { bn_apply_kernel<T, true, false, RU><<<ga, kBlk, 0, st>>>(x, res, y, coef, M, C, rpa, bits); DTG_LAUNCH_CHECK(); }
    } else {
      if (relu) { bn_apply_kernel<T, false, true, RU><<<ga, kBlk, 0, st>>>(x, res, y, coef, M, C, rpa, bits); DTG_LAUNCH_CHECK(); }
      else { bn_apply_kernel<T, false, false, RU><<<ga, kBlk, 0, st>>>(x, res, y, coef, M, C, rpa, bits); DTG_LAUNCH_CHECK(); }
    }
  }));
}

void bn_fwd_train(const bf16_t* x, const bf16_t* res, bf16_t* y, const float* gamma, const float* beta,
                  float* rmean, float* rvar, float* smean, float* sinv, float* ws, long long M, int C,
                  float momentum, float eps, int relu, hipStream_t st) {
  const BnGeom g = bn_geom(M, C);
  float* part = ws;
  float* coef = ws + (long long)g.nchunk * 2 * C;
  dim3 grid(g.nchunk, g.gy);
  DTG_TPR_SWITCH(g.tpr, bn_stats_kernel<T><<<grid, kBlk, 0, st>>>(x, M, C, g.rows_per_chunk, part)); DTG_LAUNCH_CHECK();
  bn_finalize_kernel<16><<<(C + 63) / 64, 1024, 0, st>>>(part, g.nchunk, M, C, 0, gamma, beta, rmean, rvar, smean, sinv,
                                                    momentum, eps, coef, nullptr, nullptr); DTG_LAUNCH_CHECK();
  bn_apply_launch(g, x, res, y, coef, M, C, relu, st);
}

void bn_fwd_from_part(const bf16_t* x, const bf16_t* res, bf16_t* y, const float* gamma, const float* beta,
                      float* rmean, float* rvar, float* smean, float* sinv, const float* part, float* ws, long long M,
                      int C, float momentum, float eps, int relu, hipStream_t st, uint8_t* bits) {
  const BnGeom g = bn_geom(M, C);
  bn_finalize_kernel<16><<<(C + 63) / 64, 1024, 0, st>>>(part, kBnStatSlots, M, C, 0, gamma, beta, rmean, rvar, smean,
                                                    sinv, momentum, eps, ws, nullptr, nullptr, 1); DTG_LAUNCH_CHECK();
  bn_apply_launch(g, x, res, y, ws, M, C, relu, st, bits);
}

__global__ void bn_infer_coef_kernel(const float* gamma, const float* beta, const float* rmean, const float* rvar,
                                     float eps, int C, float* coef) {
  const int c = blockIdx.x * blockDim.x + threadIdx.x;
  if (c >= C) return;
  const float inv = rsqrtf(rvar[c] + eps);
  const float sc = (gamma ? gamma[c] : 1.f) * inv;
  coef[c] = sc;
  coef[C + c] = (beta ? beta[c] : 0.f) - rmean[c] * sc;
}

void bn_fwd_infer(const bf16_t* x, const bf16_t* res, bf16_t* y, const float* gamma, const float* beta,
                  const float* rmean, const float* rvar, float* ws, long long M, int C, float eps, int relu,
                  hipStream_t st) {
  const BnGeom g = bn_geom(M, C);
  float* coef = ws;
  bn_infer_coef_kernel<<<(C + 255) / 256, 256, 0, st>>>(gamma, beta, rmean, rvar, eps, C, coef); DTG_LAUNCH_CHECK();
  dim3 grid(g.nchunk, g.gy);
  const long long rpa = elementwise_rpc(g, M);
  dim3 ga((unsigned)((M + rpa - 1) / rpa), g.gy);
  DTG_TPR_SWITCH(g.tpr, {
    if (res) {
      if (relu) { bn_apply_kernel<T, true, true><<<ga, kBlk, 0, st>>>(x, res, y, coef, M, C, rpa); DTG_LAUNCH_CHECK(); }
      else { bn_apply_kernel<T, true, false><<<ga, kBlk, 0, st>>>(x, res, y, coef, M, C, rpa); DTG_LAUNCH_CHECK(); }
    } else {
      if (relu) { bn_apply_kernel<T, false, true><<<ga, kBlk, 0, st>>>(x, res, y, coef, M, C, rpa); DTG_LAUNCH_CHECK(); }
      else { bn_apply_kernel<T, false, false><<<ga, kBlk, 0, st>>>(x, res, y, coef, M, C, rpa); DTG_LAUNCH_CHECK(); }
    }
  });
}

void bn_bwd(const bf16_t* dy, const bf16_t* y, const bf16_t* x, const float* gamma, const float* smean,
            const float* sinv, bf16_t* dx, bf16_t* dres, float* dgamma, float* dbeta, float* ws, long long M, int C,
            int relu, int accum, hipStream_t st) {
  const BnGeom g = bn_geom(M, C);
  float* part = ws;
  float* coef = ws + (long long)g.nchunk * 2 * C;
  dim3 grid(g.nchunk, g.gy);
  DTG_TPR_SWITCH(g.tpr, {
    if (relu) { bn_bwd_reduce_kernel<T, true><<<grid, kBlk, 0, st>>>(dy, y, x, smean, sinv, M, C, g.rows_per_chunk, part); DTG_LAUNCH_CHECK(); }
    else { bn_bwd_reduce_kernel<T, false><<<grid, kBlk, 0, st>>>(dy, y, x, smean, sinv, M, C, g.rows_per_chunk, part); DTG_LAUNCH_CHECK(); }
  });
  bn_finalize_kernel<16><<<(C + 63) / 64, 1024, 0, st>>>(part, g.nchunk, M, C, accum ? 2 : 1, gamma, nullptr, nullptr, nullptr,
                                                    const_cast<float*>(smean), const_cast<float*>(sinv), 0.f, 0.f,
                                                    coef, dgamma, dbeta); DTG_LAUNCH_CHECK();
  const long long rpa = elementwise_rpc(g, M);
  dim3 ga((unsigned)((M + rpa - 1) / rpa), g.gy);
  DTG_TPR_SWITCH(g.tpr, {
    if (relu) {
      if (dres) { bn_bwd_dx_kernel<T, true, true><<<ga, kBlk, 0, st>>>(dy, y, x, coef, dx, dres, M, C, rpa); DTG_LAUNCH_CHECK(); }
      else { bn_bwd_dx_kernel<T, true, false><<<ga, kBlk, 0, st>>>(dy, y, x, coef, dx, dres, M, C, rpa); DTG_LAUNCH_CHECK(); }
    } else {
      if (dres) { bn_bwd_dx_kernel<T, false, true><<<ga, kBlk, 0, st>>>(dy, y, x, coef, dx, dres, M, C, rpa); DTG_LAUNCH_CHECK(); }
      else { bn_bwd_dx_kernel<T, false, false><<<ga, kBlk, 0, st>>>(dy, y, x, coef, dx, dres, M, C, rpa); DTG_LAUNCH_CHECK(); }
    }
  });
}

void bn_fwd2_from_part(const bf16_t* x, const bf16_t* r, bf16_t* y, const float* part, const float* part2,
                       const float* gamma, const float* beta, float* rmean, float* rvar, float* smean, float* sinv,
                       const float* gamma2, const float* beta2, float* rmean2, float* rvar2, float* smean2,
                       float* sinv2, float* ws, long long M, int C, float momentum, float eps, hipStream_t st,
                       uint8_t* bits) {
  const BnGeom g = bn_geom(M, C);
  bn_finalize_kernel<16><<<(C + 63) / 64, 1024, 0, st>>>(part, kBnStatSlots, M, C, 0, gamma, beta, rmean, rvar, smean,
                                                    sinv, momentum, eps, ws, nullptr, nullptr, 1); DTG_LAUNCH_CHECK();
  bn_finalize_kernel<16><<<(C + 63) / 64, 1024, 0, st>>>(part2, kBnStatSlots, M, C, 0, gamma2, beta2, rmean2, rvar2,
                                                    smean2, sinv2, momentum, eps, ws + 2LL * C, nullptr, nullptr, 1); DTG_LAUNCH_CHECK();
  const long long rpa = elementwise_rpc(g, M);
  dim3 ga((unsigned)((M + rpa - 1) / rpa), g.gy);
  DTG_TPR_SWITCH(g.tpr, DTG_RU_SWITCH(bn_apply2_kernel<T, RU><<<ga, kBlk, 0, st>>>(x, r, y, ws, ws + 2LL * C, M, C, rpa,
                                                                                 bits))); DTG_LAUNCH_CHECK();
}

template <int TPR, int RU = 4>
__global__ void __launch_bounds__(kBlk) bn_bwd_dx2_kernel(const bf16_t* __restrict__ dp, const bf16_t* __restrict__ x,
                                                          const bf16_t* __restrict__ x2,
                                                          const float* __restrict__ coef,
                                                          const float* __restrict__ coef2, bf16_t* __restrict__ dx,
                                                          bf16_t* __restrict__ dx2, long long M, int C, long long rpc) {
  constexpr int RPP = kBlk / TPR, CW = TPR * 8;
  const int tx = threadIdx.x % TPR, ty = threadIdx.x / TPR;
  const int c0 = blockIdx.y * CW + tx * 8;
  if (c0 >= C) return;
  float a[8], bx[8], cc[8], a2[8], bx2[8], cc2[8];
  load8_f32(coef + c0, a);
  load8_f32(coef + C + c0, bx);
  load8_f32(coef + 2 * C + c0, cc);
  load8_f32(coef2 + c0, a2);
  load8_f32(coef2 + C + c0, bx2);
  load8_f32(coef2 + 2 * C + c0, cc2);
  const long long m0 = (long long)blockIdx.x * rpc;
  const long long m1 = m0 + rpc < M ? m0 + rpc : M;
  auto finish = [&](const float (&g)[8], const float (&xv)[8], const float (&x2v)[8], long long o) {
    float o1[8], o2[8];
#pragma unroll
    for (int k = 0; k < 8; ++k) {
      o1[k] = fmaf(a[k], g[k], fmaf(bx[k], xv[k], cc[k]));
      o2[k] = fmaf(a2[k], g[k], fmaf(bx2[k], x2v[k], cc2[k]));
    }
    store8_bf16(dx + o, o1);
    store8_bf16(dx2 + o, o2);
  };
  long long m = m0 + ty;
  for (; m + (RU - 1) * RPP < m1; m += RU * RPP) {
    float g[RU][8], xv[RU][8], x2v[RU][8];
#pragma unroll
    for (int u = 0; u < RU; ++u) {
      const long long o = (m + u * RPP) * C + c0;
      load8_bf16(dp + o, g[u]);
      load8_bf16(x + o, xv[u]);
      load8_bf16(x2 + o, x2v[u]);
    }
#pragma unroll
    for (int u = 0; u < RU; ++u) finish(g[u], xv[u], x2v[u], (m + u * RPP) * C + c0);
  }
  for (; m < m1; m += RPP) {
    const long long o = m * C + c0;
    float g[8], xv[8], x2v[8];
    load8_bf16(dp + o, g);
    load8_bf16(x + o, xv);
    load8_bf16(x2 + o, x2v);
    finish(g, xv, x2v, o);
  }
}

void bn_bwd2_from_part(const bf16_t* dp, const bf16_t* x, const bf16_t* x2, const float* part, const float* part2,
                       const float* gamma, const float* smean, const float* sinv, const float* gamma2,
                       const float* smean2, const float* sinv2, bf16_t* dx, bf16_t* dx2, float* dgamma, float* dbeta,
                       float* dgamma2, float* dbeta2, float* ws, long long M, int C, int accum, hipStream_t st) {
  const BnGeom g = bn_geom(M, C);
  bn_finalize_kernel<16><<<(C + 63) / 64, 1024, 0, st>>>(part, kBnStatSlots, M, C, accum ? 2 : 1, gamma, nullptr, nullptr,
                                                    nullptr, const_cast<float*>(smean), const_cast<float*>(sinv), 0.f,
                                                    0.f, ws, dgamma, dbeta, 1); DTG_LAUNCH_CHECK();
  bn_finalize_kernel<16><<<(C + 63) / 64, 1024, 0, st>>>(part2, kBnStatSlots, M, C, accum ? 2 : 1, gamma2, nullptr,
                                                    nullptr, nullptr, const_cast<float*>(smean2),
                                                    const_cast<float*>(sinv2), 0.f, 0.f, ws + 3LL * C, dgamma2,
                                                    dbeta2, 1); DTG_LAUNCH_CHECK();
  const long long rpa = elementwise_rpc(g, M);
  dim3 ga((unsigned)((M + rpa - 1) / rpa), g.gy);
  DTG_TPR_SWITCH(g.tpr, DTG_RU_SWITCH(bn_bwd_dx2_kernel<T, RU><<<ga, kBlk, 0, st>>>(dp, x, x2, ws, ws + 3LL * C, dx,
                                                                                   dx2, M, C, rpa))); DTG_LAUNCH_CHECK();
}

void bn_bwd_coef_from_part(const float* part, const float* gamma, const float* smean, const float* sinv, float* coef,
                           float* dgamma, float* dbeta, long long M, int C, int accum, hipStream_t st) {
  bn_finalize_kernel<16><<<(C + 63) / 64, 1024, 0, st>>>(part, kBnStatSlots, M, C, accum ? 2 : 1, gamma, nullptr, nullptr,
                                                    nullptr, const_cast<float*>(smean), const_cast<float*>(sinv), 0.f,
                                                    0.f, coef, dgamma, dbeta, 1); DTG_LAUNCH_CHECK();
}

void bn_dx_from_coef(const bf16_t* dp, const bf16_t* x, const float* coef, bf16_t* dx, bf16_t* dres, long long M, int C,
                     hipStream_t st) {
  const BnGeom g = bn_geom(M, C);
  const long long rpa = elementwise_rpc(g, M);
  dim3 ga((unsigned)((M + rpa - 1) / rpa), g.gy);
  const float* ws = coef;
  DTG_TPR_SWITCH(g.tpr, DTG_RU_SWITCH({
    if (dres) { bn_bwd_dx_kernel<T, false, true, true, RU><<<ga, kBlk, 0, st>>>(dp, nullptr, x, ws, dx, dres, M, C,
                                                                                      rpa); DTG_LAUNCH_CHECK(); }
    else { bn_bwd_dx_kernel<T, false, false, true, RU><<<ga, kBlk, 0, st>>>(dp, nullptr, x, ws, dx, dres, M, C, rpa); DTG_LAUNCH_CHECK(); }
  }));
}

void bn_bwd_from_part(const bf16_t* dp, const bf16_t* x, const float* gamma, const float* smean, const float* sinv,
                      const float* part, bf16_t* dx, bf16_t* dres, float* dgamma, float* dbeta, float* ws, long long M,
                      int C, int accum, hipStream_t st) {
  bn_bwd_coef_from_part(part, gamma, smean, sinv, ws, dgamma, dbeta, M, C, accum, st);
  bn_dx_from_coef(dp, x, ws, dx, dres, M, C, st);
}

}
```

csrc/kernels/bn_dx_wgrad.hip:

```cpp
#include <stdexcept>

#include "dtg/common.h"
#include "dtg/kernels.h"
#include "dtg/mfma_gemm.cuh"
#include "dtg/gemm_epi.cuh"

namespace dtg {

namespace {
using namespace gemm;

constexpr int kDC = 256;
constexpr int kDR = 32;
constexpr int kDX_LDS = kDR * kDC * 2;
constexpr int kDG_LD = 64;
constexpr int kDG_LDS = kDR * kDG_LD * 4;
constexpr int kDGW_LDS = 256 * 64 * 2;

__device__ __forceinline__ u32x4v pack8_bf16(const float (&o)[8]) {
  u32x4v w;
  w.x = pack_bf2(o[0], o[1]);
  w.y = pack_bf2(o[2], o[3]);
  w.z = pack_bf2(o[4], o[5]);
  w.w = pack_bf2(o[6], o[7]);
  return w;
}

__device__ __forceinline__ u32x4v dx_chunk(const float (&a)[8], const float (&bx)[8], const float (&cc)[8],
                                           const u32x4v& g, const u32x4v& x) {
  float gf[8], xf[8], o[8];
  unpack8_bf16(g, gf);
  unpack8_bf16(x, xf);
#pragma unroll
  for (int k = 0; k < 8; ++k) o[k] = fmaf(a[k], gf[k], fmaf(bx[k], xf[k], cc[k]));
  return pack8_bf16(o);
}

template <int CW>
__device__ __forceinline__ void store_mc_chunk(lds_char* img, int m, int c8, const u32x4v& w) {
  *reinterpret_cast<__attribute__((address_space(3))) u32x4v*>(img + m * (CW * 2) +
                                                               ((c8 ^ mc_swz<CW / 8>(m)) << 4)) = w;
}

__device__ __forceinline__ v8bf load_w_frag(const DxDgrad& dg, int ks, int wave, int lane) {
  const bf16_t* wp = dg.w + (long long)(ks * 32 + 8 * (lane >> 4)) * dg.ldw + wave * 16 + (lane & 15);
  u32x4v t;
  t.x = (uint32_t)wp[0] | ((uint32_t)wp[dg.ldw] << 16);
  t.y = (uint32_t)wp[2 * dg.ldw] | ((uint32_t)wp[3 * dg.ldw] << 16);
  t.z = (uint32_t)wp[4 * dg.ldw] | ((uint32_t)wp[5 * dg.ldw] << 16);
  t.w = (uint32_t)wp[6 * dg.ldw] | ((uint32_t)wp[7 * dg.ldw] << 16);
  return __builtin_bit_cast(v8bf, t);
}

template <int CW, int LD, class FW>
__device__ __forceinline__ void dgrad_tile(const lds_char* sdx, lds_char* sdg, int wave, int lane, FW fw) {
  const int q = lane & 15, g = lane >> 4;
  f32x4 ad[2] = {f32x4{0.f, 0.f, 0.f, 0.f}, f32x4{0.f, 0.f, 0.f, 0.f}};
#pragma unroll
  for (int ks = 0; ks < CW / 32; ++ks) {
    const v8bf w = fw(ks);
#pragma unroll
    for (int t = 0; t < 2; ++t) {
      const int m = t * 16 + q, ch = ks * 4 + g;
      const v8bf fd = *reinterpret_cast<const lds_v8bf*>(sdx + m * (CW * 2) + ((ch ^ mc_swz<CW / 8>(m)) << 4));
      ad[t] = __builtin_amdgcn_mfma_f32_16x16x32_bf16(fd, w, ad[t], 0, 0, 0);
    }
  }
  lds_float* sg = reinterpret_cast<lds_float*>(sdg);
#pragma unroll
  for (int t = 0; t < 2; ++t)
#pragma unroll
    for (int r = 0; r < 4; ++r) sg[(t * 16 + g * 4 + r) * LD + ((wave * 16 + q) ^ ((g & 1) << 4))] = ad[t][r];
}

template <int CI>
__device__ __forceinline__ void dgrad_epilogue(const lds_char* sdg, int er, int cg, const u32x4v& yv, uint32_t mb,
                                               float (&ds)[8], float (&dq)[8], bf16_t* dst) {
  const lds_float* sp = reinterpret_cast<const lds_float*>(sdg) + er * CI + ((cg * 8) ^ (((er >> 2) & 1) << 4));
  float v[8], yf[8];
#pragma unroll
  for (int k = 0; k < 8; ++k) v[k] = sp[k];
  unpack8_bf16(yv, yf);
#pragma unroll
  for (int k = 0; k < 8; ++k) {
    const float d = ((mb >> k) & 1u) ? v[k] : 0.f;
    v[k] = d;
    ds[k] += d;
    dq[k] += d * yf[k];
  }
  *reinterpret_cast<u32x4v*>(dst) = pack8_bf16(v);
}

template <int CI>
__device__ __forceinline__ void dgrad_stats_reduce(lds_float* red, int tid, int er, int cg, const float (&ds)[8],
                                                   const float (&dq)[8], const DxDgrad& dg) {
#pragma unroll
  for (int k = 0; k < 8; ++k) {
    red[er * CI + cg * 8 + k] = ds[k];
    red[(kDR + er) * CI + cg * 8 + k] = dq[k];
  }
  __syncthreads();
  if (tid < CI) {
    float ts = 0.f, tq = 0.f;
#pragma unroll 8
    for (int j = 0; j < kDR; ++j) {
      ts += red[j * CI + tid];
      tq += red[(kDR + j) * CI + tid];
    }
    tq = dg.invstd[tid] * (tq - dg.mean[tid] * ts);
    float* part = dg.part + (long long)(blockIdx.x % kBnStatSlots) * 2 * CI;
    atomicAdd(part + tid, ts);
    atomicAdd(part + CI + tid, tq);
  }
}

template <int NJ>
__device__ __forceinline__ void store_slab(float* slab, int CI, int wave, int lane, const f32x4 (&acc)[4][NJ]) {
  const int q = lane & 15, gq = lane >> 4;
#pragma unroll
  for (int i = 0; i < 4; ++i)
#pragma unroll
    for (int j = 0; j < NJ; ++j)
#pragma unroll
      for (int r = 0; r < 4; ++r) slab[(wave * 64 + i * 16 + gq * 4 + r) * CI + j * 16 + q] = acc[i][j][r];
}

template <int CI, bool DUAL, bool W2 = false, bool DG = false>
__global__ void __launch_bounds__(256, (CI == 64 && !W2) ? 2 : 1) bn_dx_wgrad_kernel(const bf16_t* __restrict__ dp, const bf16_t* __restrict__ x,
                                                          const float* __restrict__ coef,
                                                          const bf16_t* __restrict__ x2,
                                                          const float* __restrict__ coef2, bf16_t* __restrict__ dx,
                                                          bf16_t* __restrict__ dx2, const bf16_t* __restrict__ act,
                                                          long long ldact, float* __restrict__ slabs, int nblk,
                                                          int C, const bf16_t* __restrict__ act2, long long ldact2,
                                                          float* __restrict__ slabs2, DxDgrad dg) {
  static_assert(!W2 || (DUAL && CI == 64), "the second weight gradient is the dual form's, at 256 x 64");
  static_assert(!DG || (CI == 64 && DUAL == W2), "the fused dgrad is 256 x 64: the plain form or the two-weight dual");
  constexpr int kACT_LDS = kDR * CI * 2;
  constexpr int NJ = CI / 16;
  constexpr int NX = W2 ? 2 : 1;
  constexpr bool WLDS = DG && !W2;
  __shared__ __attribute__((aligned(16))) char smem_raw[NX * (kDX_LDS + 2 * kACT_LDS) + (DG ? kDG_LDS : 0) +
                                                        (WLDS ? kDGW_LDS : 0)];
  lds_char* sdx = (lds_char*)smem_raw;
  lds_char* sact = sdx + kDX_LDS;
  lds_char* sdx2 = sact + 2 * kACT_LDS;
  lds_char* sact2 = sdx2 + kDX_LDS;
  lds_char* sdg = (lds_char*)smem_raw + NX * (kDX_LDS + 2 * kACT_LDS);
  const int tid = threadIdx.x, lane = tid & 63;
  const int wave = __builtin_amdgcn_readfirstlane(tid >> 6);
  const int G = gridDim.x;
  const int ns = C / kDC, gid = xcd_remap(blockIdx.x, G);
  const int sl = gid % ns;
  const int c8 = tid & 31, rs = tid >> 5, c0 = sl * kDC + c8 * 8;
  float a[8], bx[8], cc[8], a2[8], bx2[8], cc2[8];
  load8_f32(coef + c0, a);
  load8_f32(coef + C + c0, bx);
  load8_f32(coef + 2 * C + c0, cc);
  if constexpr (DUAL) {
    load8_f32(coef2 + c0, a2);
    load8_f32(coef2 + C + c0, bx2);
    load8_f32(coef2 + 2 * C + c0, cc2);
  }
  DenseMC<false> sa{act, ldact, CI, 0};
  DenseMC<false> sa2{act2, ldact2, CI, 0};
  f32x4 acc[4][NJ], acc2[W2 ? 4 : 1][W2 ? NJ : 1];
#pragma unroll
  for (int i = 0; i < 4; ++i)
#pragma unroll
    for (int j = 0; j < NJ; ++j) acc[i][j] = f32x4{0.f, 0.f, 0.f, 0.f};
  if constexpr (W2) {
#pragma unroll
    for (int i = 0; i < 4; ++i)
#pragma unroll
      for (int j = 0; j < NJ; ++j) acc2[i][j] = f32x4{0.f, 0.f, 0.f, 0.f};
  }
  v8bf wf[(DG && !WLDS) ? 8 : 1];
  lds_v8bf* swf = reinterpret_cast<lds_v8bf*>(sdg + kDG_LDS) + wave * 8 * 64 + lane;
  float ds[8] = {0, 0, 0, 0, 0, 0, 0, 0}, dq[8] = {0, 0, 0, 0, 0, 0, 0, 0};
  const int er = tid >> 3, cg = tid & 7;
  if constexpr (DG) {
#pragma unroll
    for (int ks = 0; ks < 8; ++ks) {
      const v8bf t = load_w_frag(dg, ks, wave, lane);
      if constexpr (WLDS) swf[ks * 64] = t;
      else wf[ks] = t;
    }
  }

  u32x4v g[4], xv[4], x2v[4];
  u32x4v yv, yvn;
  uint32_t mb, mbn;
  auto issue = [&](int b, int slot) {
    const long long m0 = (long long)b * kDR;
    if constexpr (DG) {
      yvn = *reinterpret_cast<const u32x4v*>(dg.y + (m0 + er) * CI + cg * 8);
      mbn = dg.bits[(m0 + er) * (CI / 8) + cg];
    }
    stage_mc<CI, DenseMC<false>, 4, kDR>(sa, sact + slot * kACT_LDS, 0, (int)m0, wave, lane);
    if constexpr (W2) stage_mc<CI, DenseMC<false>, 4, kDR>(sa2, sact2 + slot * kACT_LDS, 0, (int)m0, wave, lane);
#pragma unroll
    for (int u = 0; u < 4; ++u) {
      const long long off = (m0 + rs + 8 * u) * C + c0;
      g[u] = *reinterpret_cast<const u32x4v*>(dp + off);
      xv[u] = *reinterpret_cast<const u32x4v*>(x + off);
      if constexpr (DUAL) x2v[u] = *reinterpret_cast<const u32x4v*>(x2 + off);
    }
  };
  const int b0 = gid / ns, gb = G / ns;
  if (b0 < nblk) issue(b0, 0);
  int slot = 0;
  for (int b = b0; b < nblk; b += gb, slot ^= 1) {
    const long long m0 = (long long)b * kDR;
    if constexpr (DG) {
      yv = yvn;
      mb = mbn;
    }
#pragma unroll
    for (int u = 0; u < 4; ++u) {
      const int m = rs + 8 * u;
      const long long off = (m0 + m) * C + c0;
      const u32x4v w = dx_chunk(a, bx, cc, g[u], xv[u]);
      if constexpr (!DG) *reinterpret_cast<u32x4v*>(dx + off) = w;
      store_mc_chunk<kDC>(sdx, m, c8, w);
      if constexpr (DUAL) {
        const u32x4v w2 = dx_chunk(a2, bx2, cc2, g[u], x2v[u]);
        *reinterpret_cast<u32x4v*>(dx2 + off) = w2;
        if constexpr (W2) store_mc_chunk<kDC>(sdx2, m, c8, w2);
      }
    }
    const bool more = b + gb < nblk;
    if (more) issue(b + gb, slot ^ 1);
    constexpr int PIECES = (CI / 64) * (W2 ? 2 : 1);
    constexpr int NST = (DG ? 0 : 4) + (DUAL ? 4 : 0), NLD = (DUAL ? 12 : 8) + (DG ? 2 : 0);
    if (more) asm volatile("s_waitcnt vmcnt(%0) lgkmcnt(0)" ::"n"(NST + PIECES + NLD) : "memory");
    else asm volatile("s_waitcnt vmcnt(%0) lgkmcnt(0)" ::"n"(NST) : "memory");
    __builtin_amdgcn_s_barrier();
    v8bf fa[4], fb[NJ];
#pragma unroll
    for (int i = 0; i < 4; ++i) fa[i] = frag_mc<kDC>(sdx, wave * 64 + i * 16, 0, lane);
#pragma unroll
    for (int j = 0; j < NJ; ++j) fb[j] = frag_mc<CI>(sact + slot * kACT_LDS, j * 16, 0, lane);
#pragma unroll
    for (int i = 0; i < 4; ++i)
#pragma unroll
      for (int j = 0; j < NJ; ++j)
        acc[i][j] = __builtin_amdgcn_mfma_f32_16x16x32_bf16(fa[i], fb[j], acc[i][j], 0, 0, 0);
    if constexpr (W2) {
#pragma unroll
      for (int i = 0; i < 4; ++i) fa[i] = frag_mc<kDC>(sdx2, wave * 64 + i * 16, 0, lane);
#pragma unroll
      for (int j = 0; j < NJ; ++j) fb[j] = frag_mc<CI>(sact2 + slot * kACT_LDS, j * 16, 0, lane);
#pragma unroll
      for (int i = 0; i < 4; ++i)
#pragma unroll
        for (int j = 0; j < NJ; ++j)
          acc2[i][j] = __builtin_amdgcn_mfma_f32_16x16x32_bf16(fa[i], fb[j], acc2[i][j], 0, 0, 0);
    }
    if constexpr (DG)
      dgrad_tile<kDC, CI>(sdx, sdg, wave, lane, [&](int ks) -> v8bf {
        if constexpr (WLDS) return swf[ks * 64];
        else return wf[ks];
      });
    asm volatile("s_waitcnt lgkmcnt(0)" ::: "memory");
    __builtin_amdgcn_s_barrier();
    if constexpr (DG) dgrad_epilogue<CI>(sdg, er, cg, yv, mb, ds, dq, dg.dp + (m0 + er) * CI + cg * 8);
  }
  asm volatile("s_waitcnt vmcnt(0)" ::: "memory");
  if constexpr (DG) {
    if (b0 < nblk) dgrad_stats_reduce<CI>(reinterpret_cast<lds_float*>(sdx), tid, er, cg, ds, dq, dg);
  }
  store_slab<NJ>(slabs + ((long long)(gid / ns) * C + sl * kDC) * CI, CI, wave, lane, acc);
  if constexpr (W2) store_slab<NJ>(slabs2 + ((long long)(gid / ns) * C + sl * kDC) * CI, CI, wave, lane, acc2);
}

constexpr int kFC = 512, kFCI = 128;
constexpr int kFW_REG = 5;
constexpr int kFDX_LDS = kDR * kFC * 2;
constexpr int kFACT_LDS = kDR * kFCI * 2;
constexpr int kFDG_LDS = kDR * kFCI * 4;
constexpr int kFCOEF_LDS = 3 * kFC * 4;
constexpr int kFW_LDS = (16 - kFW_REG) * 32 * kFCI * 2;
constexpr int kF_LDS = kFDX_LDS + kFACT_LDS + kFDG_LDS + kFCOEF_LDS + kFW_LDS;

__global__ void __launch_bounds__(512, 1) bn_dx_wgrad_full_kernel(const bf16_t* __restrict__ dp, const bf16_t* __restrict__ x,
                                                                  const float* __restrict__ coef,
                                                                  const bf16_t* __restrict__ act, long long ldact,
                                                                  float* __restrict__ slabs, int nblk, DxDgrad dg) {
  constexpr int C = kFC, CI = kFCI, NJ = CI / 16, KS = C / 32;
  extern __shared__ __attribute__((aligned(16))) char smem_dyn[];
  lds_char* sdx = (lds_char*)smem_dyn;
  lds_char* sact = sdx + kFDX_LDS;
  lds_char* sdg = sact + kFACT_LDS;
  lds_float* scoef = reinterpret_cast<lds_float*>(sdg + kFDG_LDS);
  const int tid = threadIdx.x, lane = tid & 63;
  const int wave = __builtin_amdgcn_readfirstlane(tid >> 6);
  const int G = gridDim.x, gid = xcd_remap(blockIdx.x, G);
  f32x4 acc[4][NJ];
#pragma unroll
  for (int i = 0; i < 4; ++i)
#pragma unroll
    for (int j = 0; j < NJ; ++j) acc[i][j] = f32x4{0.f, 0.f, 0.f, 0.f};
  v8bf wf[kFW_REG];
  lds_v8bf* swf = reinterpret_cast<lds_v8bf*>(scoef + 3 * C) + wave * (KS - kFW_REG) * 64 + lane;
  float ds[8] = {0, 0, 0, 0, 0, 0, 0, 0}, dq[8] = {0, 0, 0, 0, 0, 0, 0, 0};
#pragma unroll
  for (int ks = 0; ks < KS; ++ks) {
    const v8bf t = load_w_frag(dg, ks, wave, lane);
    if (ks < kFW_REG) wf[ks < kFW_REG ? ks : 0] = t;
    else swf[(ks - kFW_REG) * 64] = t;
  }
  for (int i = tid; i < 3 * C; i += 512) scoef[i] = coef[i];
  __syncthreads();

  auto load8_lds = [](const lds_float* p, float (&o)[8]) {
    const f32x4 lo = *reinterpret_cast<const __attribute__((address_space(3))) f32x4*>(p);
    const f32x4 hi = *reinterpret_cast<const __attribute__((address_space(3))) f32x4*>(p + 4);
    o[0] = lo[0]; o[1] = lo[1]; o[2] = lo[2]; o[3] = lo[3]; o[4] = hi[0]; o[5] = hi[1]; o[6] = hi[2]; o[7] = hi[3];
  };
  u32x4v g[4], xv[4], av;
  auto issue = [&](int b, int t) {
    const long long m0 = (long long)b * kDR;
    av = *reinterpret_cast<const u32x4v*>(act + (m0 + (t >> 4)) * ldact + (t & 15) * 8);
#pragma unroll
    for (int u = 0; u < 4; ++u) {
      const long long off = (m0 + (t >> 6) + 8 * u) * C + (t & 63) * 8;
      g[u] = *reinterpret_cast<const u32x4v*>(dp + off);
      xv[u] = *reinterpret_cast<const u32x4v*>(x + off);
    }
  };
  if (gid < nblk) issue(gid, tid);
  for (int b = gid; b < nblk; b += G) {
    const long long m0 = (long long)b * kDR;
    int tl = tid;
    asm volatile("" : "+v"(tl));
    const int c8 = tl & 63, rs = tl >> 6, c0 = c8 * 8, er = tl >> 4, cg = tl & 15;
    const u32x4v yv = *reinterpret_cast<const u32x4v*>(dg.y + (m0 + er) * CI + cg * 8);
    const uint32_t mb = dg.bits[(m0 + er) * (CI / 8) + cg];
    {
      float a[8], bx[8], cc[8];
      load8_lds(scoef + c0, a);
      load8_lds(scoef + C + c0, bx);
      load8_lds(scoef + 2 * C + c0, cc);
      store_mc_chunk<CI>(sact, er, cg, av);
#pragma unroll
      for (int u = 0; u < 4; ++u)
        store_mc_chunk<C>(sdx, rs + 8 * u, c8, dx_chunk(a, bx, cc, g[u], xv[u]));
    }
    issue(b + G < nblk ? b + G : b, tl);
    asm volatile("s_waitcnt lgkmcnt(0)" ::: "memory");
    __builtin_amdgcn_s_barrier();
    const int ln = tl & 63;
    {
      v8bf fa[4];
#pragma unroll
      for (int i = 0; i < 4; ++i) fa[i] = frag_mc<C>(sdx, wave * 64 + i * 16, 0, ln);
#pragma unroll
      for (int j = 0; j < NJ; ++j) {
        const v8bf fb = frag_mc<CI>(sact, j * 16, 0, ln);
#pragma unroll
        for (int i = 0; i < 4; ++i) acc[i][j] = __builtin_amdgcn_mfma_f32_16x16x32_bf16(fa[i], fb, acc[i][j], 0, 0, 0);
      }
    }
    dgrad_tile<C, CI>(sdx, sdg, wave, ln, [&](int ks) -> v8bf {
      if (ks < kFW_REG) return wf[ks < kFW_REG ? ks : 0];
      return swf[(ks - kFW_REG) * 64];
    });
    asm volatile("s_waitcnt lgkmcnt(0)" ::: "memory");
    __builtin_amdgcn_s_barrier();
    dgrad_epilogue<CI>(sdg, er, cg, yv, mb, ds, dq, dg.dp + (m0 + er) * CI + cg * 8);
  }
  if (gid < nblk) dgrad_stats_reduce<CI>(reinterpret_cast<lds_float*>(sdx), tid, tid >> 4, tid & 15, ds, dq, dg);
  store_slab<NJ>(slabs + (long long)gid * C * CI, CI, wave, lane, acc);
}

struct DxForm {
  void (*launch)(const DxForm& f, hipStream_t st, const bf16_t* dp, const DxSide& a, const DxSide& b, int nblk, int C,
                 const DxDgrad& d);
  int block, lds, grid, slabs;
};

int persistent_grid(const void* kern, int block, int lds, int cap) {
  int dev = 0, cus = 0, per_cu = 0;
  DTG_HIP_CHECK(hipGetDevice(&dev));
  DTG_HIP_CHECK(hipDeviceGetAttribute(&cus, hipDeviceAttributeMultiprocessorCount, dev));
  if (lds) DTG_HIP_CHECK(hipFuncSetAttribute(kern, hipFuncAttributeMaxDynamicSharedMemorySize, lds));
  DTG_HIP_CHECK(hipOccupancyMaxActiveBlocksPerMultiprocessor(&per_cu, kern, block, lds));
  if (lds && per_cu < 1) throw std::runtime_error("bn_dx_wgrad: the full-width form does not fit a CU");
  int G = cus * (per_cu < 1 ? 1 : (per_cu > cap ? cap : per_cu));
  G -= G % 8;
  return G < 8 ? 8 : G;
}

template <int CI, bool DUAL, bool W2 = false, bool DG = false>
DxForm sliced_form(int C) {
  static const int G = persistent_grid((const void*)bn_dx_wgrad_kernel<CI, DG ? W2 : true, W2, DG>, 256, 0, 2);
  return {[](const DxForm& f, hipStream_t st, const bf16_t* dp, const DxSide& a, const DxSide& b, int nblk, int C,
             const DxDgrad& d) {
            hipLaunchKernelGGL((bn_dx_wgrad_kernel<CI, DUAL, W2, DG>), dim3(f.grid), dim3(f.block), f.lds, st, dp, a.x,
                               a.coef, b.x, b.coef, a.dx, b.dx, a.act, a.ldact, a.slabs, nblk, C, b.act, b.ldact,
                               b.slabs, d);
          },
          256, 0, G, G / (C / kDC)};
}

DxForm full_form() {
  static const int G = persistent_grid((const void*)bn_dx_wgrad_full_kernel, 512, kF_LDS, 1);
  return {[](const DxForm& f, hipStream_t st, const bf16_t* dp, const DxSide& a, const DxSide&, int nblk, int,
             const DxDgrad& d) {
            hipLaunchKernelGGL(bn_dx_wgrad_full_kernel, dim3(f.grid), dim3(f.block), f.lds, st, dp, a.x, a.coef, a.act,
                               a.ldact, a.slabs, nblk, d);
          },
          512, kF_LDS, G, G};
}

DxForm dx_form(int C, int CI, bool dual, bool w2, bool dg) {
  if (dg && C == kFC) {
    if (CI != kFCI || dual || w2)
      throw std::invalid_argument("bn_dx_wgrad: the full-width fused dgrad is 512 x 128, plain form");
    return full_form();
  }
  if (dg) {
    if (C != 256 || CI != 64 || dual != w2)
      throw std::invalid_argument("bn_dx_wgrad: the fused dgrad is 256 x 64, plain or two-weight dual form");
    return w2 ? sliced_form<64, true, true, true>(C) : sliced_form<64, false, false, true>(C);
  }
  if (w2) {
    if (C != 256 || CI != 64 || !dual)
      throw std::invalid_argument("bn_dx_wgrad: the second weight gradient is the dual form's, at 256 x 64");
    return sliced_form<64, true, true>(C);
  }
  if (C == 256 && CI == 64) return dual ? sliced_form<64, true>(C) : sliced_form<64, false>(C);
  if (C == 512 && CI == 128) return dual ? sliced_form<128, true>(C) : sliced_form<128, false>(C);
  throw std::invalid_argument("bn_dx_wgrad: 256 x 64 or 512 x 128 (bn_dx_wgrad_ok)");
}

}

bool bn_dx_wgrad_ok(long long M, int C, int CI) {
  return ((C == 256 && CI == 64) || (C == 512 && CI == 128)) && M % kDR == 0 && M >= 64LL * kDR;
}

bool bn_dx_dgrad_ok(long long M, int C, int CI) { return C == 256 && CI == 64 && bn_dx_wgrad_ok(M, C, CI); }

bool bn_dx_dgrad_full_ok(long long M, int C, int CI) { return C == kFC && CI == kFCI && bn_dx_wgrad_ok(M, C, CI); }

int bn_dx_wgrad_slabs(int C, int CI, int w2, int dg) { return dx_form(C, CI, w2 != 0, w2 != 0, dg != 0).slabs; }

void bn_dx_wgrad(const bf16_t* dp, const DxSide& main, const DxSide* second, long long M, int C, int CI,
                 int wgrad_bf16, hipStream_t st, const DxDgrad* dg) {
  if (!bn_dx_wgrad_ok(M, C, CI)) throw std::invalid_argument("bn_dx_wgrad: unsupported shape (bn_dx_wgrad_ok)");
  const DxSide b = second ? *second : DxSide{};
  const DxForm f = dx_form(C, CI, b.x != nullptr, b.act != nullptr, dg != nullptr);
  f.launch(f, st, dp, main, b, (int)(M / kDR), C, dg ? *dg : DxDgrad{});
  DTG_LAUNCH_CHECK();
  for (const DxSide* s : {&b, &main})
    if (s->act) {
      Epi e{s->wgrad, CI, wgrad_bf16, 1.f, 1.f, nullptr, 0};
      gemm_splitk_reduce(s->slabs, f.slabs, C, CI, e, st);
    }
}

}
```

distributed-tensorflow-guide_amd/models/resnet.py:

```python
import torch
import torch.nn as nn

from . import resnet_fused
from ..ops.pool import max_pool2d, global_avg_pool
from .layers import ConvBN, Linear


class Bottleneck(nn.Module):
    expansion = 4

    def __init__(self, cin, width, stride=1):
        super().__init__()
        cout = width * self.expansion
        self.c1 = ConvBN(cin, width, 1)
        self.c2 = ConvBN(width, width, 3, stride, 1)
        self.c3 = ConvBN(width, cout, 1, zero_init=True)
        self.down = ConvBN(cin, cout, 1, stride) if (stride != 1 or cin != cout) else None

    fused = True

    def forward(self, x):
        if self.fused and resnet_fused.fused_ok(self, x):
            return resnet_fused.bottleneck(self, x)
        idn = self.down(x, relu=False) if self.down is not None else x
        y = self.c1(x)
        y = self.c2(y)
        return self.c3(y, residual=idn, relu=True)


class ResNet(nn.Module):
    def __init__(self, layers=(3, 4, 6, 3), num_classes=1000, width=64):
        super().__init__()
        self.stem = ConvBN(3, width, 7, 2, 3)
        blocks = []
        cin = width
        for i, n in enumerate(layers):
            w = width * (2 ** i)
            for j in range(n):
                blocks.append(Bottleneck(cin, w, stride=2 if (j == 0 and i > 0) else 1))
                cin = w * Bottleneck.expansion
        self.blocks = nn.Sequential(*blocks)
        self.fc = Linear(cin, num_classes, init_std=0.01)

    def forward(self, x):
        if resnet_fused.stem_ok(self.stem, x):
            x = resnet_fused.stem_pool(self.stem, x)
        else:
            x = self.stem(x)
            x = max_pool2d(x, 3, 2, 1)
        x = self.blocks(x)
        x = global_avg_pool(x)
        return self.fc(x)


def resnet50(num_classes=1000):
    return ResNet((3, 4, 6, 3), num_classes)


def resnet18_like_tiny(num_classes=10):
    return ResNet((1, 1, 1, 1), num_classes, width=8)


def synthetic_batch(batch, device, dtype=torch.bfloat16, image=224, num_classes=1000, seed=0):
    g = torch.Generator(device="cpu").manual_seed(seed)
    x = torch.randn(batch, 3, image, image, generator=g).to(device=device, dtype=dtype)
    x = x.contiguous(memory_format=torch.channels_last)
    y = torch.randint(0, num_classes, (batch,), generator=g).to(device)
    return x, y
```

distributed-tensorflow-guide_amd/models/resnet_fused.py:

```python
import os

import torch
import torch.nn.functional as F

from ..ops import conv as conv_ops
from ..ops._native import lib
from ..ops.gemm import gemm
from ..parallel import grad_sink, overlap


def _rows(t):
    n, c, h, w = t.shape
    if not t.is_contiguous(memory_format=torch.channels_last):
        t = t.contiguous(memory_format=torch.channels_last)
    return t.permute(0, 2, 3, 1).reshape(n * h * w, c)


def _mat(w):
    return w.reshape(w.shape[0], w.shape[1]) if w.is_contiguous() else w.as_strided((w.shape[0], w.shape[1]),
                                                                                     (w.shape[1], 1))


def _krsc(w):
    return w.permute(0, 2, 3, 1)


_FUSE = True
_LINK = True
_SUB2 = True
_DXW = True
_DXW2 = True
_DXD = True
_DXD2 = True
_DXD_S2 = True
_dxd_calls = 0


class _Bn3Link:
    __slots__ = ("y3", "m3", "i3", "gamma", "beta", "bits", "yd", "md", "idd", "part", "part2", "dp")

    def __init__(self, y3, m3, i3, gamma, beta, bits, yd=None, md=None, idd=None):
        self.y3, self.m3, self.i3, self.gamma, self.beta = y3, m3, i3, gamma, beta
        self.bits = bits
        self.yd, self.md, self.idd = yd, md, idd
        self.part = self.part2 = self.dp = None


def _gacc(p):
    if grad_sink.enabled(p):
        return p.grad, True
    return torch.zeros_like(p, dtype=torch.float32 if p.dim() <= 1 else p.dtype), False


_BITS = True


_WSPLIT_WGS = int(os.environ.get("DTG_RESNET_WSPLIT_WGS", "256"))
_CWSPLIT_WGS = int(os.environ.get("DTG_RESNET_CWSPLIT_WGS", "256"))
_wsplit_cache = {}


def _wgrad(dy, x, out):
    tgt = _WSPLIT_WGS if overlap.enabled() else 0
    key = (dy.shape[1], x.shape[1], dy.shape[0], tgt)
    sk = _wsplit_cache.get(key)
    if sk is None:
        sk = _wsplit_cache[key] = lib().gemm_pick_split(key[0], key[1], key[2], False, tgt) if tgt > 0 else 0
    gemm(dy, False, x, False, out=out, beta=1.0, split_k=sk)


def _conv_wgrad(dy4, x4, dw, st, pad):
    lib().conv_wgrad(dy4, x4, dw, 1.0, st, pad, target_wgs=_CWSPLIT_WGS if overlap.enabled() else 0)


def _relu_bits(y):
    return torch.empty(y.shape[0], y.shape[1] // 8, device=y.device, dtype=torch.uint8) if _BITS else None


class _BottleneckFn(torch.autograd.Function):
    @staticmethod
    def forward(ctx, x, blk, link_in, holder, *params):
        L = lib()
        n, c, h, w = x.shape
        st = blk.c2.conv.stride
        width = blk.c1.conv.weight.shape[0]
        cout = blk.c3.conv.weight.shape[0]
        x2 = _rows(x)
        p_, q_ = (h + 2 - 3) // st + 1, (w + 2 - 3) // st + 1
        b1, b2, b3 = blk.c1.bn, blk.c2.bn, blk.c3.bn
        w1, w2, w3 = blk.c1.conv.weight, blk.c2.conv.weight, blk.c3.conv.weight
        if _FUSE:
            y1, p1 = L.gemm_bn(x2, _mat(w1), 1, pooled=True)
            bits1 = _relu_bits(y1)
            a1, m1, i1 = L.bn_fwd_part(y1, p1, None, b1.weight, b1.bias, b1.running_mean, b1.running_var,
                                       b1.momentum, b1.eps, True, bits=bits1)
            y2, p2 = L.conv_fwd_bn(a1.view(n, h, w, width), _krsc(w2), st, 1, pooled=True)
            y2 = y2.view(-1, width)
            bits2 = _relu_bits(y2)
            a2, m2, i2 = L.bn_fwd_part(y2, p2, None, b2.weight, b2.bias, b2.running_mean, b2.running_var,
                                       b2.momentum, b2.eps, True, bits=bits2)
            y3, p3 = L.gemm_bn(a2, _mat(w3), 1, pooled=True)
            ctx.bits12 = (bits1, bits2)
        else:
            y1 = gemm(x2, True, _mat(w1), True)
            a1, m1, i1 = L.bn_fwd_train(y1, None, b1.weight, b1.bias, b1.running_mean, b1.running_var, b1.momentum,
                                        b1.eps, True)
            y2 = L.conv_fwd(a1.view(n, h, w, width), _krsc(w2), st, 1).view(-1, width)
            a2, m2, i2 = L.bn_fwd_train(y2, None, b2.weight, b2.bias, b2.running_mean, b2.running_var, b2.momentum,
                                        b2.eps, True)
            y3 = gemm(a2, True, _mat(w3), True)
        yd = md = idd = None
        if blk.down is not None:
            bd, wd = blk.down.bn, blk.down.conv.weight
            if _FUSE:
                if st == 1:
                    yd, pd = L.gemm_bn(x2, _mat(wd), 1, pooled=True)
                else:
                    yd, pd = L.conv_fwd_bn(x2.view(n, h, w, c), _krsc(wd), st, 0, pooled=True)
                    yd = yd.view(-1, cout)
                idn = None
            else:
                if st == 1:
                    yd = gemm(x2, True, _mat(wd), True)
                else:
                    yd = L.conv_fwd(x2.view(n, h, w, c), _krsc(wd), st, 0).view(-1, cout)
                idn, md, idd = L.bn_fwd_train(yd, None, bd.weight, bd.bias, bd.running_mean, bd.running_var,
                                              bd.momentum, bd.eps, False)
        else:
            idn = x2
        bits = None
        if _FUSE and _LINK:
            bits = torch.empty(y3.shape[0], cout // 8, device=y3.device, dtype=torch.uint8)
        if _FUSE and blk.down is not None:
            assert bd.momentum == b3.momentum and bd.eps == b3.eps
            out, m3, i3, md, idd = L.bn_fwd2_part(y3, p3, b3.weight, b3.bias, b3.running_mean, b3.running_var, yd, pd,
                                                  bd.weight, bd.bias, bd.running_mean, bd.running_var, b3.momentum,
                                                  b3.eps, bits=bits)
        elif _FUSE:
            out, m3, i3 = L.bn_fwd_part(y3, p3, idn, b3.weight, b3.bias, b3.running_mean, b3.running_var,
                                        b3.momentum, b3.eps, True, bits=bits)
        else:
            out, m3, i3 = L.bn_fwd_train(y3, idn, b3.weight, b3.bias, b3.running_mean, b3.running_var, b3.momentum,
                                         b3.eps, True)
        ctx.blk = blk
        ctx.link_in = link_in if (_FUSE and _LINK) else None
        ctx.link_out = _Bn3Link(y3, m3, i3, b3.weight, b3.bias, bits, yd, md, idd) if (_FUSE and _LINK) else None
        holder.append(ctx.link_out)
        ctx.geom = (n, c, h, w, st, width, cout, p_, q_)
        ctx.save_for_backward(x2, y1, a1, m1, i1, y2, a2, m2, i2, y3, out, m3, i3,
                              *((yd, md, idd) if yd is not None else ()))
        return out.view(n, p_, q_, cout).permute(0, 3, 1, 2)

    @staticmethod
    def backward(ctx, dout):
        L = lib()
        blk = ctx.blk
        n, c, h, w, st, width, cout, p_, q_ = ctx.geom
        sv = ctx.saved_tensors
        x2, y1, a1, m1, i1, y2, a2, m2, i2, y3, out, m3, i3 = sv[:13]
        b1, b2, b3 = blk.c1.bn, blk.c2.bn, blk.c3.bn
        w1, w2, w3 = blk.c1.conv.weight, blk.c2.conv.weight, blk.c3.conv.weight
        params = [w1, b1.weight, b1.bias, w2, b2.weight, b2.bias, w3, b3.weight, b3.bias]
        if blk.down is not None:
            params += [blk.down.conv.weight, blk.down.bn.weight, blk.down.bn.bias]
        accs = [_gacc(p) for p in params]
        g = {id(p): a for p, (a, _) in zip(params, accs)}
        do = _rows(dout)
        lk = ctx.link_out
        dyd = None
        w3_kw = (dict(wact=a2, wgrad=g[id(w3)].view(cout, width))
                 if _DXW and a2 is not None and L.bn_dx_wgrad_ok(y3.shape[0], cout, width) else None)
        w3_done = wd_done = False
        bits1, bits2 = ctx.bits12 if _FUSE else (None, None)
        ctx.bits12 = None
        dp2 = q2 = None
        dxd = (_DXD and w3_kw is not None and bits2 is not None and L.bn_dx_dgrad_ok(y3.shape[0], cout, width))
        dxd_full = (_DXD_S2 and w3_kw is not None and bits2 is not None
                    and L.bn_dx_dgrad_full_ok(y3.shape[0], cout, width))

        def dg_kw(full=False):
            return dict(dgw=_mat(w3), dgy=y2, dgmean=m2, dginv=i2, dgbits=bits2,
                        dgpart=L.bn_part_alloc(y2, width, pooled=True), dgfull=full)
        if (lk is not None and lk.part is not None and do.data_ptr() == lk.dp.data_ptr()
                and do.shape == lk.dp.shape):
            if lk.part2 is not None:
                bd = blk.down.bn
                kw = dict(w3_kw or {})
                if _DXW2 and w3_kw is not None and st == 1 and c == width == 64 and cout == 256:
                    kw.update(wact2=x2, wgrad2=g[id(blk.down.conv.weight)].view(cout, c))
                    wd_done = True
                dxd = dxd and wd_done and _DXD2
                if dxd:
                    kw.update(dg_kw())
                r = L.bn_bwd2_part(do, y3, lk.part, b3.weight, m3, i3, g[id(b3.weight)], g[id(b3.bias)],
                                   sv[13], lk.part2, bd.weight, sv[14], sv[15], g[id(bd.weight)],
                                   g[id(bd.bias)], **kw)
                dy3, dyd = r[0], r[1]
                if dxd:
                    dp2, q2 = r[2], r[3]
                w3_done = w3_kw is not None
            else:
                kw = dict(w3_kw or {})
                dxd = dxd or dxd_full
                if dxd:
                    kw.update(dg_kw(dxd_full))
                r = L.bn_bwd_part(do, y3, lk.part, b3.weight, m3, i3, False, g[id(b3.weight)], g[id(b3.bias)], **kw)
                dy3 = r[0]
                if dxd:
                    dp2, q2 = r[4], r[5]
                w3_done = w3_kw is not None
            if dp2 is not None:
                global _dxd_calls
                _dxd_calls += 1
            dres = do
        else:
            for pt in ((lk.part, lk.part2) if lk is not None else ()):
                if pt is not None:
                    pt.zero_()
            dy3, dres, _, _ = L.bn_bwd(do, out, y3, b3.weight, m3, i3, True, True, g[id(b3.weight)],
                                       g[id(b3.bias)])
        if lk is not None:
            lk.part = lk.part2 = lk.dp = None
        if dp2 is not None:
            pass
        elif _FUSE and bits2 is not None:
            dp2, q2 = L.gemm_bn(dy3, _mat(w3), 3, y2, m2, i2, b2.weight, b2.bias, mask=bits2, pooled=True)
        elif _FUSE:
            dp2, q2 = L.gemm_bn(dy3, _mat(w3), 2, y2, m2, i2, b2.weight, b2.bias, pooled=True)
        else:
            da2 = gemm(dy3, True, _mat(w3), False)
        if w3_done:
            pass
        else:
            with overlap.wgrad_scope(dy3, a2):
                _wgrad(dy3, a2, g[id(w3)].view(cout, width))
        if _FUSE:
            dy2 = L.bn_bwd_part(dp2, y2, q2, b2.weight, m2, i2, False, g[id(b2.weight)], g[id(b2.bias)])[0]
        else:
            dy2 = L.bn_bwd(da2, a2, y2, b2.weight, m2, i2, True, False, g[id(b2.weight)], g[id(b2.bias)])[0]
        dy2_4 = dy2.view(n, p_, q_, width)
        if _FUSE:
            dp1, q1 = L.conv_dgrad_bn(dy2_4, _krsc(w2).contiguous(), h, w, st, 1, y1, m1, i1, b1.weight, b1.bias,
                                       pooled=True, bits=bits1)
            dp1 = dp1.view(-1, width)
        else:
            da1 = L.conv_dgrad(dy2_4, _krsc(w2).contiguous(), h, w, st, 1).view(-1, width)
        with overlap.wgrad_scope(dy2_4, a1):
            _conv_wgrad(dy2_4, a1.view(n, h, w, width), g[id(w2)].permute(0, 2, 3, 1), st, 1)
        dx_done = False
        sub2_hw = None
        lk_in = ctx.link_in
        ctx.link_in = None
        if lk_in is not None and lk_in.y3.shape != x2.shape:
            lk_in = None
        if _FUSE:
            dy1 = L.bn_bwd_part(dp1, y1, q1, b1.weight, m1, i1, False, g[id(b1.weight)], g[id(b1.bias)])[0]
        else:
            dy1 = L.bn_bwd(da1, a1, y1, b1.weight, m1, i1, True, False, g[id(b1.weight)], g[id(b1.bias)])[0]
        if blk.down is not None:
            yd, md, idd = sv[13:16]
            bd, wd = blk.down.bn, blk.down.conv.weight
            if dyd is None:
                dyd, _, _, _ = L.bn_bwd(dres, None, yd, bd.weight, md, idd, False, False, g[id(bd.weight)],
                                        g[id(bd.bias)])
            if st == 1:
                dx2 = gemm(dyd, True, _mat(wd), False)
                if not wd_done:
                    with overlap.wgrad_scope(dyd, x2):
                        _wgrad(dyd, x2, g[id(wd)].view(cout, c))
            elif lk_in is not None:
                sub2 = st == 2 and _SUB2
                dx2 = L.conv_dgrad(dyd.view(n, p_, q_, cout), _krsc(wd).contiguous(), h, w, st, 0,
                                   zero_rest=not sub2).view(-1, c)
                if sub2:
                    sub2_hw = (h, w)
                with overlap.wgrad_scope(dyd, x2):
                    _conv_wgrad(dyd.view(n, p_, q_, cout), x2.view(n, h, w, c), g[id(wd)].permute(0, 2, 3, 1), st, 0)
            else:
                dx2 = gemm(dy1, True, _mat(w1), False)
                L.conv_dgrad(dyd.view(n, p_, q_, cout), _krsc(wd).contiguous(), h, w, st, 0, out=dx2.view(n, h, w, c),
                             beta=1.0)
                dx_done = True
                with overlap.wgrad_scope(dyd, x2):
                    _conv_wgrad(dyd.view(n, p_, q_, cout), x2.view(n, h, w, c), g[id(wd)].permute(0, 2, 3, 1), st, 0)
        else:
            dx2 = dres
        if not dx_done:
            if lk_in is not None:
                part2 = None
                if lk_in.yd is not None:
                    part2 = L.bn_part_alloc(dp1, c, pooled=True)
                _, part = L.gemm_bn(dy1, _mat(w1), 3, lk_in.y3, lk_in.m3, lk_in.i3, lk_in.gamma, lk_in.beta,
                                    mask=lk_in.bits, out=dx2, pooled=True, x2=lk_in.yd, mean2=lk_in.md,
                                    invstd2=lk_in.idd, part2=part2, sub2_hw=sub2_hw)
                lk_in.part, lk_in.part2, lk_in.dp = part, part2, dx2
            else:
                gemm(dy1, True, _mat(w1), False, out=dx2, beta=1.0)
        with overlap.wgrad_scope(dy1, x2):
            _wgrad(dy1, x2, g[id(w1)].view(width, c))
        if not all(direct for _, direct in accs):
            overlap.sync_current(x2.device)
        grads = []
        for p, (a, direct) in zip(params, accs):
            if direct:
                grad_sink.notify(p)
                grads.append(None)
            else:
                grads.append(a.to(p.dtype))
        return (dx2.view(n, h, w, c).permute(0, 3, 1, 2), None, None, None, *grads)


def fused_ok(blk, x):
    ws = [blk.c1.conv.weight, blk.c2.conv.weight, blk.c3.conv.weight]
    return (blk.training and x.is_cuda and x.dtype == torch.bfloat16 and all(v.dtype == torch.bfloat16 for v in ws)
            and x.shape[1] % 64 == 0 and blk.c1.conv.weight.shape[0] % 64 == 0)


def bottleneck(blk, x):
    params = [blk.c1.conv.weight, blk.c1.bn.weight, blk.c1.bn.bias, blk.c2.conv.weight, blk.c2.bn.weight,
              blk.c2.bn.bias, blk.c3.conv.weight, blk.c3.bn.weight, blk.c3.bn.bias]
    if blk.down is not None:
        params += [blk.down.conv.weight, blk.down.bn.weight, blk.down.bn.bias]
    holder = []
    y = _BottleneckFn.apply(x, blk, getattr(x, "_dtg_bn3", None), holder, *params)
    if holder and holder[0] is not None:
        y._dtg_bn3 = holder[0]
    return y


_STEM = True
_POOL = (3, 2, 1)
_STEM_YAM = True
_STEM_WG_SCHED = 3
_STEM_WG_WGS = 512


class _StemFn(torch.autograd.Function):
    @staticmethod
    def forward(ctx, x, stem, w, gamma, beta):
        L = lib()
        n, c, h, wd = x.shape
        conv, bn = stem.conv, stem.bn
        k, _, r, s = w.shape
        st, pad = conv.stride, conv.padding
        if conv_ops.stem_pairs_ok(x, w, st):
            x8, w8, (rk, sk) = conv_ops.stem_pairs(x, w, st, pad)
            y4, part = L.conv_fwd_c8(x8, w8, rk, sk, st, 0, True, stride_w=1)
            ctx.pairs = True
        else:
            ctx.pairs = False
            x8 = F.pad(x.permute(0, 2, 3, 1), (0, 8 - c)).contiguous()
            w8 = F.pad(w.permute(0, 2, 3, 1), (0, 8 - c)).reshape(k, r * s * 8)
            kp = (r * s * 8 + 63) // 64 * 64
            w8 = F.pad(w8, (0, kp - r * s * 8)).contiguous()
            y4, part = L.conv_fwd_c8(x8, w8, r, s, st, pad, True)
        yam_ok = _STEM_YAM and L.stem_pooled_stats_ok(y4.shape[-1])
        res = L.stem_bn_pool_fwd(y4, part, gamma, beta, bn.running_mean, bn.running_var, bn.momentum, bn.eps,
                                 *_POOL, save_yam=yam_ok)
        out, idx, smean, sinv = res[:4]
        ctx.save_for_backward(x8, y4, idx, smean, sinv, res[4] if yam_ok else None)
        ctx.stem = stem
        ctx.geom = (c, k, r, s, st, pad)
        return out.permute(0, 3, 1, 2)

    @staticmethod
    def backward(ctx, dout):
        L = lib()
        x8, y4, idx, smean, sinv, yam = ctx.saved_tensors
        c, k, r, s, st, pad = ctx.geom
        stem = ctx.stem
        w, gamma, beta = stem.conv.weight, stem.bn.weight, stem.bn.bias
        (dg, dg_direct), (db, db_direct) = _gacc(gamma), _gacc(beta)
        do4 = dout.contiguous(memory_format=torch.channels_last).permute(0, 2, 3, 1)
        dy4 = L.stem_bn_pool_bwd(do4, idx, y4, gamma, beta, smean, sinv, *_POOL, dgamma_acc=dg, dbeta_acc=db,
                                 yam=yam)[0]
        if ctx.pairs:
            dwp = torch.empty(k, r, (s + 1) // 2, 8, device=x8.device, dtype=torch.float32)
            L.conv_wgrad(dy4, x8, dwp, 0.0, st, 0, stride_w=1, sched=_STEM_WG_SCHED,
                         target_wgs=_STEM_WG_WGS)
        else:
            dwp = torch.empty(k, r, s, 8, device=x8.device, dtype=torch.float32)
            L.conv_wgrad(dy4, x8, dwp, 0.0, st, pad)
        grads = []
        if grad_sink.enabled(w):
            L.stem_dw_add(dwp, w.grad, ctx.pairs)
            grad_sink.notify(w)
            grads.append(None)
        else:
            dw = conv_ops.stem_pairs_dw(dwp, c, s) if ctx.pairs else dwp[..., :c].permute(0, 3, 1, 2)
            grads.append(dw.to(w.dtype).contiguous(memory_format=torch.channels_last))
        for p, (a, direct) in ((gamma, (dg, dg_direct)), (beta, (db, db_direct))):
            if direct:
                grad_sink.notify(p)
                grads.append(None)
            else:
                grads.append(a.to(p.dtype))
        return (None, None, *grads)


def stem_ok(stem, x):
    w = stem.conv.weight
    return (_STEM and stem.training and x.is_cuda and x.dtype == torch.bfloat16 and not x.requires_grad
            and w.dtype == torch.bfloat16 and x.shape[1] <= 8 and w.shape[0] % 64 == 0
            and x.is_contiguous(memory_format=torch.channels_last))


def stem_pool(stem, x):
    return _StemFn.apply(x, stem, stem.conv.weight, stem.bn.weight, stem.bn.bias)
```

Measured before the change: 17360 images/sec.

## Fuse block-output BN apply with the next block's conv1 GEMM

The final BN+residual+ReLU apply of a bottleneck now also computes the next block's 1x1 conv1 GEMM and its BN partial statistics in one kernel. This applies for stage-1 and stage-2 shapes. The next block then consumes the precomputed output instead of re-reading the activation for its own conv1 GEMM. This is meant to cut one full activation read and a kernel launch per block boundary. In exchange it adds a stateful handoff object between blocks, validated by pointer and weight-version checks, plus shape-restricted kernel templates.

```diff
diff --git a/csrc/bindings/ops.cc b/csrc/bindings/ops.cc
--- a/csrc/bindings/ops.cc
+++ b/csrc/bindings/ops.cc
@@ -1033,9 +1033,33 @@
   check_f32(ts, (long long)dtg::kBnStatSlots * 2 * C, "partials");
 }
 
-std::tuple<Tensor, Tensor, Tensor> bn_fwd_part(Tensor x, Tensor part, c10::optional<Tensor> res, Tensor gamma,
-                                               Tensor beta, Tensor rmean, Tensor rvar, double momentum, double eps,
-                                               bool relu, c10::optional<Tensor> bits) {
+static bool next_conv(const c10::optional<Tensor>& nw, const c10::optional<Tensor>& npart, const Tensor& x, bool form_ok,
+                      bool two, dtg::BnNextConv& nx, Tensor& y1n) {
+  if (!nw.has_value() || !nw->defined()) return false;
+  const long long M = x.size(0);
+  const int C = (int)x.size(1);
+  CHECK_CUDA(*nw);
+  CHECK_DT(*nw, at::kBFloat16);
+  TORCH_CHECK(nw->dim() == 2 && nw->size(1) == C && nw->stride(1) == 1 && nw->stride(0) % 8 == 0 &&
+                  ((uintptr_t)nw->data_ptr() % 16) == 0,
+              "next weight must be [N, C] with 16-byte aligned rows");
+  const int N = (int)nw->size(0);
+  TORCH_CHECK(form_ok && dtg::bn_apply_gemm_ok(M, C, N) && !(two && C == 256 && N != 64),
+              "bn_apply_gemm: unsupported shape or form (bn_apply_gemm_ok)");
+  TORCH_CHECK(npart.has_value() && npart->defined(), "next weight needs next_part");
+  check_f32({&*npart}, (long long)dtg::kBnStatSlots * 2 * N, "next_part");
+  y1n = at::empty({M, N}, x.options());
+  nx.w = cbfp(*nw);
+  nx.ldw = nw->stride(0);
+  nx.N = N;
+  nx.y = bfp(y1n);
+  nx.part = npart->data_ptr<float>();
+  return true;
+}
+
+pybind11::tuple bn_fwd_part(Tensor x, Tensor part, c10::optional<Tensor> res, Tensor gamma, Tensor beta, Tensor rmean,
+                            Tensor rvar, double momentum, double eps, bool relu, c10::optional<Tensor> bits,
+                            c10::optional<Tensor> next_w, c10::optional<Tensor> next_part) {
   CHECK_IN(x);
   CHECK_DT(x, at::kBFloat16);
   TORCH_CHECK(x.dim() == 2, "x must be [M, C]");
@@ -1051,21 +1075,25 @@
     TORCH_CHECK(res->sizes() == x.sizes(), "residual shape mismatch");
   }
   c10::DeviceGuard dg(x.device());
+  dtg::BnNextConv nx;
+  Tensor y1n;
+  const bool fuse = next_conv(next_w, next_part, x, has_res && relu, false, nx, y1n);
   auto y = at::empty_like(x);
   auto fopt = x.options().dtype(at::kFloat);
   auto smean = at::empty({C}, fopt), sinv = at::empty({C}, fopt), ws = at::empty({2LL * C}, fopt);
   dtg::bn_fwd_from_part(cbfp(x), has_res ? cbfp(*res) : nullptr, bfp(y), gamma.data_ptr<float>(),
                         beta.data_ptr<float>(), rmean.data_ptr<float>(), rvar.data_ptr<float>(),
                         smean.data_ptr<float>(), sinv.data_ptr<float>(), part.data_ptr<float>(), ws.data_ptr<float>(),
-                        M, C, (float)momentum, (float)eps, relu, cur_stream(), bits_ptr(bits, M, C));
-  return {y, smean, sinv};
-}
-
-std::tuple<Tensor, Tensor, Tensor, Tensor, Tensor> bn_fwd2_part(Tensor x, Tensor part, Tensor gamma, Tensor beta,
-                                                                Tensor rmean, Tensor rvar, Tensor r, Tensor part2,
-                                                                Tensor gamma2, Tensor beta2, Tensor rmean2,
-                                                                Tensor rvar2, double momentum, double eps,
-                                                                c10::optional<Tensor> bits) {
+                        M, C, (float)momentum, (float)eps, relu, cur_stream(), bits_ptr(bits, M, C),
+                        fuse ? &nx : nullptr);
+  if (fuse) return pybind11::make_tuple(y, smean, sinv, y1n);
+  return pybind11::make_tuple(y, smean, sinv);
+}
+
+pybind11::tuple bn_fwd2_part(Tensor x, Tensor part, Tensor gamma, Tensor beta, Tensor rmean, Tensor rvar, Tensor r,
+                             Tensor part2, Tensor gamma2, Tensor beta2, Tensor rmean2, Tensor rvar2, double momentum,
+                             double eps, c10::optional<Tensor> bits, c10::optional<Tensor> next_w,
+                             c10::optional<Tensor> next_part) {
   CHECK_IN(x);
   CHECK_IN(r);
   CHECK_DT(x, at::kBFloat16);
@@ -1077,6 +1105,9 @@
   check_partials({&part, &part2}, C);
   check_per_channel({&gamma, &beta, &rmean, &rvar, &gamma2, &beta2, &rmean2, &rvar2}, C);
   c10::DeviceGuard dg(x.device());
+  dtg::BnNextConv nx;
+  Tensor y1n;
+  const bool fuse = next_conv(next_w, next_part, x, true, true, nx, y1n);
   auto y = at::empty_like(x);
   auto fopt = x.options().dtype(at::kFloat);
   auto m1 = at::empty({C}, fopt), i1 = at::empty({C}, fopt), m2 = at::empty({C}, fopt), i2 = at::empty({C}, fopt);
@@ -1086,8 +1117,9 @@
                          rvar.data_ptr<float>(), m1.data_ptr<float>(), i1.data_ptr<float>(), gamma2.data_ptr<float>(),
                          beta2.data_ptr<float>(), rmean2.data_ptr<float>(), rvar2.data_ptr<float>(),
                          m2.data_ptr<float>(), i2.data_ptr<float>(), ws.data_ptr<float>(), M, C, (float)momentum,
-                         (float)eps, cur_stream(), bits_ptr(bits, M, C));
-  return {y, m1, i1, m2, i2};
+                         (float)eps, cur_stream(), bits_ptr(bits, M, C), fuse ? &nx : nullptr);
+  if (fuse) return pybind11::make_tuple(y, m1, i1, m2, i2, y1n);
+  return pybind11::make_tuple(y, m1, i1, m2, i2);
 }
 
 static void check_wgrad_fuse(const Tensor& x, const c10::optional<Tensor>& wact, const c10::optional<Tensor>& wgrad) {
@@ -1355,13 +1387,19 @@
   m.def("bn_fwd2_part", &bn_fwd2_part, pybind11::arg("x"), pybind11::arg("part"), pybind11::arg("gamma"),
         pybind11::arg("beta"), pybind11::arg("rmean"), pybind11::arg("rvar"), pybind11::arg("r"), pybind11::arg("part2"),
         pybind11::arg("gamma2"), pybind11::arg("beta2"), pybind11::arg("rmean2"), pybind11::arg("rvar2"),
-        pybind11::arg("momentum"), pybind11::arg("eps"), pybind11::arg("bits") = pybind11::none());
+        pybind11::arg("momentum"), pybind11::arg("eps"), pybind11::arg("bits") = pybind11::none(),
+        pybind11::arg("next_w") = pybind11::none(), pybind11::arg("next_part") = pybind11::none());
+  m.def("bn_apply_gemm_ok", [](int64_t M, int64_t C, int64_t N) { return dtg::bn_apply_gemm_ok(M, (int)C, (int)N); });
+  m.def("bn_apply_gemm_grid",
+        [](int64_t C, int64_t N, bool two) { return dtg::bn_apply_gemm_grid((int)C, (int)N, two); },
+        pybind11::arg("C"), pybind11::arg("N"), pybind11::arg("two") = false);
   m.def("conv_fwd_c8", &conv_fwd_c8, pybind11::arg("x"), pybind11::arg("w"), pybind11::arg("R"), pybind11::arg("S"),
         pybind11::arg("stride"), pybind11::arg("pad"), pybind11::arg("with_stats") = false,
         pybind11::arg("stride_w") = 0);
   m.def("bn_fwd_part", &bn_fwd_part, pybind11::arg("x"), pybind11::arg("part"), pybind11::arg("res"),
         pybind11::arg("gamma"), pybind11::arg("beta"), pybind11::arg("rmean"), pybind11::arg("rvar"),
-        pybind11::arg("momentum"), pybind11::arg("eps"), pybind11::arg("relu"), pybind11::arg("bits") = pybind11::none());
+        pybind11::arg("momentum"), pybind11::arg("eps"), pybind11::arg("relu"), pybind11::arg("bits") = pybind11::none(),
+        pybind11::arg("next_w") = pybind11::none(), pybind11::arg("next_part") = pybind11::none());
   m.def("bn_bwd_part", &bn_bwd_part, pybind11::arg("dp"), pybind11::arg("x"), pybind11::arg("part"),
         pybind11::arg("gamma"), pybind11::arg("smean"), pybind11::arg("sinv"), pybind11::arg("want_dres"),
         pybind11::arg("dgamma_acc") = pybind11::none(), pybind11::arg("dbeta_acc") = pybind11::none(),
diff --git a/csrc/include/dtg/bn_apply_expr.cuh b/csrc/include/dtg/bn_apply_expr.cuh
--- /dev/null
+++ b/csrc/include/dtg/bn_apply_expr.cuh
@@ -0,0 +1,43 @@
+#pragma once
+#include "dtg/common.h"
+
+namespace dtg {
+
+template <bool RES, bool RELU>
+__device__ __forceinline__ void bn_apply8(float (&a)[8], const float (&r)[8], const float (&sc)[8],
+                                          const float (&sf)[8]) {
+#pragma unroll
+  for (int k = 0; k < 8; ++k) {
+    float v = a[k] * sc[k] + sf[k];
+    if constexpr (RES) v += r[k];
+    if constexpr (RELU) v = fmaxf(v, 0.f);
+    a[k] = v;
+  }
+}
+
+__device__ __forceinline__ void bn_apply2_8(float (&a)[8], const float (&b)[8], const float (&sc)[8],
+                                            const float (&sc2)[8], const float (&sf)[8]) {
+#pragma unroll
+  for (int k = 0; k < 8; ++k) a[k] = fmaxf(fmaf(a[k], sc[k], fmaf(b[k], sc2[k], sf[k])), 0.f);
+}
+
+__device__ __forceinline__ uint8_t pos_bits8(const float (&v)[8]) {
+  uint32_t b = 0;
+#pragma unroll
+  for (int k = 0; k < 8; ++k) b |= (v[k] > 0.f ? 1u : 0u) << k;
+  return (uint8_t)b;
+}
+
+__device__ __forceinline__ void store_bits(uint8_t* bits, long long off, const float (&v)[8], int tx, int C) {
+  const uint32_t b = pos_bits8(v);
+  if ((C & 31) == 0) {
+    uint32_t w = b << (8 * (tx & 3));
+    w |= __shfl_xor(w, 1, 64);
+    w |= __shfl_xor(w, 2, 64);
+    if ((tx & 3) == 0) *reinterpret_cast<uint32_t*>(bits + (off >> 3)) = w;
+  } else {
+    bits[off >> 3] = (uint8_t)b;
+  }
+}
+
+}
diff --git a/csrc/include/dtg/kernels.h b/csrc/include/dtg/kernels.h
--- a/csrc/include/dtg/kernels.h
+++ b/csrc/include/dtg/kernels.h
@@ -113,14 +113,26 @@
 }
 
 long long bn_workspace_floats(long long M, int C);
+struct BnNextConv {
+  const bf16_t* w = nullptr;
+  long long ldw = 0;
+  int N = 0;
+  bf16_t* y = nullptr;
+  float* part = nullptr;
+};
+bool bn_apply_gemm_ok(long long M, int C, int N);
+int bn_apply_gemm_grid(int C, int N, int two);
+void bn_apply_gemm(const bf16_t* x, const bf16_t* r, const float* coef, const float* coef2, bf16_t* out,
+                   uint8_t* bits, const BnNextConv& next, long long M, int C, hipStream_t st);
 void bn_fwd_from_part(const bf16_t* x, const bf16_t* res, bf16_t* y, const float* gamma, const float* beta,
                       float* rmean, float* rvar, float* smean, float* sinv, const float* part, float* ws, long long M,
-                      int C, float momentum, float eps, int relu, hipStream_t st, uint8_t* bits = nullptr);
+                      int C, float momentum, float eps, int relu, hipStream_t st, uint8_t* bits = nullptr,
+                      const BnNextConv* next = nullptr);
 void bn_fwd2_from_part(const bf16_t* x, const bf16_t* r, bf16_t* y, const float* part, const float* part2,
                        const float* gamma, const float* beta, float* rmean, float* rvar, float* smean, float* sinv,
                        const float* gamma2, const float* beta2, float* rmean2, float* rvar2, float* smean2,
                        float* sinv2, float* ws, long long M, int C, float momentum, float eps, hipStream_t st,
-                       uint8_t* bits = nullptr);
+                       uint8_t* bits = nullptr, const BnNextConv* next = nullptr);
 void bn_bwd2_from_part(const bf16_t* dp, const bf16_t* x, const bf16_t* x2, const float* part, const float* part2,
                        const float* gamma, const float* smean, const float* sinv, const float* gamma2,
                        const float* smean2, const float* sinv2, bf16_t* dx, bf16_t* dx2, float* dgamma, float* dbeta,
diff --git a/csrc/kernels/batchnorm.hip b/csrc/kernels/batchnorm.hip
--- a/csrc/kernels/batchnorm.hip
+++ b/csrc/kernels/batchnorm.hip
@@ -2,6 +2,7 @@
 #include "dtg/common.h"
 #include "dtg/kernels.h"
 #include "dtg/bn_finalize.cuh"
+#include "dtg/bn_apply_expr.cuh"
 
 namespace dtg {
 
@@ -51,25 +52,6 @@
   }
 }
 
-__device__ __forceinline__ uint8_t pos_bits8(const float (&v)[8]) {
-  uint32_t b = 0;
-#pragma unroll
-  for (int k = 0; k < 8; ++k) b |= (v[k] > 0.f ? 1u : 0u) << k;
-  return (uint8_t)b;
-}
-
-__device__ __forceinline__ void store_bits(uint8_t* bits, long long off, const float (&v)[8], int tx, int C) {
-  const uint32_t b = pos_bits8(v);
-  if ((C & 31) == 0) {
-    uint32_t w = b << (8 * (tx & 3));
-    w |= __shfl_xor(w, 1, 64);
-    w |= __shfl_xor(w, 2, 64);
-    if ((tx & 3) == 0) *reinterpret_cast<uint32_t*>(bits + (off >> 3)) = w;
-  } else {
-    bits[off >> 3] = (uint8_t)b;
-  }
-}
-
 template <int TPR, bool RES, bool RELU, int RU = 4>
 __global__ void __launch_bounds__(kBlk) bn_apply_kernel(const bf16_t* __restrict__ x, const bf16_t* __restrict__ res,
                                                         bf16_t* __restrict__ y, const float* __restrict__ coef,
@@ -85,13 +67,7 @@
   const long long m0 = (long long)blockIdx.x * rpc;
   const long long m1 = m0 + rpc < M ? m0 + rpc : M;
   auto finish = [&](float (&a)[8], const float (&r)[8], long long off) {
-#pragma unroll
-    for (int k = 0; k < 8; ++k) {
-      float v = a[k] * sc[k] + sf[k];
-      if constexpr (RES) v += r[k];
-      if constexpr (RELU) v = fmaxf(v, 0.f);
-      a[k] = v;
-    }
+    bn_apply8<RES, RELU>(a, r, sc, sf);
     store8_bf16(y + off, a);
     if (bits) store_bits(bits, off, a, tx, C);
   };
@@ -134,8 +110,7 @@
   const long long m0 = (long long)blockIdx.x * rpc;
   const long long m1 = m0 + rpc < M ? m0 + rpc : M;
   auto finish = [&](float (&a)[8], const float (&b)[8], long long o) {
-#pragma unroll
-    for (int k = 0; k < 8; ++k) a[k] = fmaxf(fmaf(a[k], sc[k], fmaf(b[k], sc2[k], sf[k])), 0.f);
+    bn_apply2_8(a, b, sc, sc2, sf);
     store8_bf16(y + o, a);
     if (bits) store_bits(bits, o, a, tx, C);
   };
@@ -310,10 +285,13 @@
 
 void bn_fwd_from_part(const bf16_t* x, const bf16_t* res, bf16_t* y, const float* gamma, const float* beta,
                       float* rmean, float* rvar, float* smean, float* sinv, const float* part, float* ws, long long M,
-                      int C, float momentum, float eps, int relu, hipStream_t st, uint8_t* bits) {
+                      int C, float momentum, float eps, int relu, hipStream_t st, uint8_t* bits,
+                      const BnNextConv* next) {
+  if (next && !(res && relu)) throw std::invalid_argument("bn_fwd_from_part: the next conv needs the residual + relu form");
   const BnGeom g = bn_geom(M, C);
   bn_finalize_kernel<16><<<(C + 63) / 64, 1024, 0, st>>>(part, kBnStatSlots, M, C, 0, gamma, beta, rmean, rvar, smean,
                                                     sinv, momentum, eps, ws, nullptr, nullptr, 1); DTG_LAUNCH_CHECK();
+  if (next) return bn_apply_gemm(x, res, ws, nullptr, y, bits, *next, M, C, st);
   bn_apply_launch(g, x, res, y, ws, M, C, relu, st, bits);
 }
 
@@ -378,12 +356,13 @@
                        const float* gamma, const float* beta, float* rmean, float* rvar, float* smean, float* sinv,
                        const float* gamma2, const float* beta2, float* rmean2, float* rvar2, float* smean2,
                        float* sinv2, float* ws, long long M, int C, float momentum, float eps, hipStream_t st,
-                       uint8_t* bits) {
+                       uint8_t* bits, const BnNextConv* next) {
   const BnGeom g = bn_geom(M, C);
   bn_finalize_kernel<16><<<(C + 63) / 64, 1024, 0, st>>>(part, kBnStatSlots, M, C, 0, gamma, beta, rmean, rvar, smean,
                                                     sinv, momentum, eps, ws, nullptr, nullptr, 1); DTG_LAUNCH_CHECK();
   bn_finalize_kernel<16><<<(C + 63) / 64, 1024, 0, st>>>(part2, kBnStatSlots, M, C, 0, gamma2, beta2, rmean2, rvar2,
                                                     smean2, sinv2, momentum, eps, ws + 2LL * C, nullptr, nullptr, 1); DTG_LAUNCH_CHECK();
+  if (next) return bn_apply_gemm(x, r, ws, ws + 2LL * C, y, bits, *next, M, C, st);
   const long long rpa = elementwise_rpc(g, M);
   dim3 ga((unsigned)((M + rpa - 1) / rpa), g.gy);
   DTG_TPR_SWITCH(g.tpr, DTG_RU_SWITCH(bn_apply2_kernel<T, RU><<<ga, kBlk, 0, st>>>(x, r, y, ws, ws + 2LL * C, M, C, rpa,
diff --git a/csrc/kernels/bn_dx_wgrad.hip b/csrc/kernels/bn_dx_wgrad.hip
--- a/csrc/kernels/bn_dx_wgrad.hip
+++ b/csrc/kernels/bn_dx_wgrad.hip
@@ -4,6 +4,7 @@
 #include "dtg/kernels.h"
 #include "dtg/mfma_gemm.cuh"
 #include "dtg/gemm_epi.cuh"
+#include "dtg/bn_apply_expr.cuh"
 
 namespace dtg {
 
@@ -374,6 +375,122 @@
   store_slab<NJ>(slabs + (long long)gid * C * CI, CI, wave, lane, acc);
 }
 
+template <int C, int N, bool TWO>
+__global__ void __launch_bounds__(C, C == 256 ? 2 : 1) bn_apply_gemm_kernel(const bf16_t* __restrict__ x, const bf16_t* __restrict__ r,
+                                                               const float* __restrict__ coef,
+                                                               const float* __restrict__ coef2,
+                                                               bf16_t* __restrict__ out, uint8_t* __restrict__ bits,
+                                                               const bf16_t* __restrict__ w1, long long ldw,
+                                                               bf16_t* __restrict__ y1n, float* __restrict__ part,
+                                                               int nblk) {
+  static_assert((C == 256 && (N == 64 || N == 128)) || (C == 512 && N == 128),
+                "conv1 of stage 1 (64), of stage 2's first block (128), or of stage 2 (512 x 128)");
+  constexpr int NTH = C, NT = N / 16 / (NTH / 64), KS = C / 32;
+  constexpr int CG = N / 8, NR = NTH / CG, NP = kDR / NR;
+  constexpr int kIMG_LDS = kDR * C * 2;
+  constexpr int kTILE_LDS = kDR * N * 4;
+  static_assert(2 * NR * N * 4 <= kIMG_LDS, "the statistics reduction goes through the out image");
+  __shared__ __attribute__((aligned(16))) char smem_raw[kIMG_LDS + kTILE_LDS];
+  lds_char* simg = (lds_char*)smem_raw;
+  lds_char* stile = simg + kIMG_LDS;
+  const int tid = threadIdx.x, lane = tid & 63;
+  const int wave = __builtin_amdgcn_readfirstlane(tid >> 6);
+  const int G = gridDim.x, gid = xcd_remap(blockIdx.x, G);
+  const int c8 = tid % (C / 8), rs = tid / (C / 8), c0 = c8 * 8;
+  float sc[8], sf[8], sc2[8];
+  load8_f32(coef + c0, sc);
+  load8_f32(coef + C + c0, sf);
+  if constexpr (TWO) {
+    float sf2[8];
+    load8_f32(coef2 + c0, sc2);
+    load8_f32(coef2 + C + c0, sf2);
+#pragma unroll
+    for (int k = 0; k < 8; ++k) sf[k] += sf2[k];
+  }
+  v8bf wf[NT][KS];
+#pragma unroll
+  for (int h = 0; h < NT; ++h)
+#pragma unroll
+    for (int ks = 0; ks < KS; ++ks)
+      wf[h][ks] = *reinterpret_cast<const v8bf*>(w1 + (long long)((wave * NT + h) * 16 + (lane & 15)) * ldw + ks * 32 +
+                                                 8 * (lane >> 4));
+  float ss[8] = {0, 0, 0, 0, 0, 0, 0, 0}, sq[8] = {0, 0, 0, 0, 0, 0, 0, 0};
+  const int er0 = tid / CG, cg = tid % CG;
+
+  u32x4v xv[4], rv[4];
+  auto issue = [&](int b) {
+    const long long m0 = (long long)b * kDR;
+#pragma unroll
+    for (int u = 0; u < 4; ++u) {
+      const long long off = (m0 + rs + 8 * u) * C + c0;
+      xv[u] = *reinterpret_cast<const u32x4v*>(x + off);
+      rv[u] = *reinterpret_cast<const u32x4v*>(r + off);
+    }
+  };
+  if (gid < nblk) issue(gid);
+  for (int b = gid; b < nblk; b += G) {
+    const long long m0 = (long long)b * kDR;
+#pragma unroll
+    for (int u = 0; u < 4; ++u) {
+      const int m = rs + 8 * u;
+      const long long off = (m0 + m) * C + c0;
+      float a[8], rf[8];
+      unpack8_bf16(xv[u], a);
+      unpack8_bf16(rv[u], rf);
+      if constexpr (TWO) bn_apply2_8(a, rf, sc, sc2, sf);
+      else bn_apply8<true, true>(a, rf, sc, sf);
+      const u32x4v w = pack8_bf16(a);
+      *reinterpret_cast<u32x4v*>(out + off) = w;
+      if (bits) store_bits(bits, off, a, c8, C);
+      store_mc_chunk<C>(simg, m, c8, w);
+    }
+    issue(b + G < nblk ? b + G : b);
+    asm volatile("s_waitcnt lgkmcnt(0)" ::: "memory");
+    __builtin_amdgcn_s_barrier();
+#pragma unroll
+    for (int h = 0; h < NT; ++h)
+      dgrad_tile<C, N>(simg, stile, wave * NT + h, lane, [&](int ks) -> v8bf { return wf[h][ks]; });
+    asm volatile("s_waitcnt lgkmcnt(0)" ::: "memory");
+    __builtin_amdgcn_s_barrier();
+#pragma unroll
+    for (int p = 0; p < NP; ++p) {
+      const int er = er0 + p * NR;
+      const lds_float* sp = reinterpret_cast<const lds_float*>(stile) + er * N + ((cg * 8) ^ (((er >> 2) & 1) << 4));
+      float v[8], rd[8];
+#pragma unroll
+      for (int k = 0; k < 8; ++k) v[k] = sp[k];
+      const u32x4v w = pack8_bf16(v);
+      unpack8_bf16(w, rd);
+#pragma unroll
+      for (int k = 0; k < 8; ++k) {
+        ss[k] += rd[k];
+        sq[k] += rd[k] * rd[k];
+      }
+      *reinterpret_cast<u32x4v*>(y1n + (m0 + er) * N + cg * 8) = w;
+    }
+  }
+  if (gid < nblk) {
+    lds_float* red = reinterpret_cast<lds_float*>(simg);
+#pragma unroll
+    for (int k = 0; k < 8; ++k) {
+      red[er0 * N + cg * 8 + k] = ss[k];
+      red[(NR + er0) * N + cg * 8 + k] = sq[k];
+    }
+    __syncthreads();
+    if (tid < N) {
+      float ts = 0.f, tq = 0.f;
+#pragma unroll 8
+      for (int j = 0; j < NR; ++j) {
+        ts += red[j * N + tid];
+        tq += red[(NR + j) * N + tid];
+      }
+      float* slot = part + (long long)(gid % kBnStatSlots) * 2 * N;
+      atomicAdd(slot + tid, ts);
+      atomicAdd(slot + N + tid, tq);
+    }
+  }
+}
+
 struct DxForm {
   void (*launch)(const DxForm& f, hipStream_t st, const bf16_t* dp, const DxSide& a, const DxSide& b, int nblk, int C,
                  const DxDgrad& d);
@@ -461,4 +578,46 @@
     }
 }
 
-}
+namespace {
+struct ApplyGemmForm {
+  int grid;
+  void (*launch)(int grid, hipStream_t st, const bf16_t* x, const bf16_t* r, const float* coef, const float* coef2,
+                 bf16_t* out, uint8_t* bits, const BnNextConv& nx, int nblk);
+};
+
+template <int C, int N, bool TWO>
+ApplyGemmForm apply_gemm_form_of() {
+  static const int G = persistent_grid((const void*)bn_apply_gemm_kernel<C, N, TWO>, C, 0, C == 256 ? 2 : 1);
+  return {G, [](int grid, hipStream_t st, const bf16_t* x, const bf16_t* r, const float* coef, const float* coef2,
+                bf16_t* out, uint8_t* bits, const BnNextConv& nx, int nblk) {
+            hipLaunchKernelGGL((bn_apply_gemm_kernel<C, N, TWO>), dim3(grid), dim3(C), 0, st, x, r, coef, coef2, out,
+                               bits, nx.w, nx.ldw, nx.y, nx.part, nblk);
+          }};
+}
+
+ApplyGemmForm apply_gemm_form(int C, int N, bool two) {
+  if (C == 256 && N == 64) return two ? apply_gemm_form_of<256, 64, true>() : apply_gemm_form_of<256, 64, false>();
+  if (C == 256 && N == 128 && !two) return apply_gemm_form_of<256, 128, false>();
+  if (C == 512 && N == 128) return two ? apply_gemm_form_of<512, 128, true>() : apply_gemm_form_of<512, 128, false>();
+  throw std::invalid_argument("bn_apply_gemm: 256 x 64, 256 x 128 (residual form) or 512 x 128 (bn_apply_gemm_ok)");
+}
+}
+
+bool bn_apply_gemm_ok(long long M, int C, int N) {
+  return ((C == 256 && (N == 64 || N == 128)) || (C == 512 && N == 128)) && M % kDR == 0 && M >= 64LL * kDR &&
+         M / kDR < (1LL << 31);
+}
+
+int bn_apply_gemm_grid(int C, int N, int two) { return apply_gemm_form(C, N, two != 0).grid; }
+
+void bn_apply_gemm(const bf16_t* x, const bf16_t* r, const float* coef, const float* coef2, bf16_t* out,
+                   uint8_t* bits, const BnNextConv& next, long long M, int C, hipStream_t st) {
+  if (!bn_apply_gemm_ok(M, C, next.N)) throw std::invalid_argument("bn_apply_gemm: unsupported shape (bn_apply_gemm_ok)");
+  if (!r || !next.w || !next.y || !next.part || next.ldw < C || next.ldw % 8)
+    throw std::invalid_argument("bn_apply_gemm: missing operand or unaligned weight rows");
+  const ApplyGemmForm f = apply_gemm_form(C, next.N, coef2 != nullptr);
+  f.launch(f.grid, st, x, r, coef, coef2, out, bits, next, (int)(M / kDR));
+  DTG_LAUNCH_CHECK();
+}
+
+}
diff --git a/distributed-tensorflow-guide_amd/models/resnet.py b/distributed-tensorflow-guide_amd/models/resnet.py
--- a/distributed-tensorflow-guide_amd/models/resnet.py
+++ b/distributed-tensorflow-guide_amd/models/resnet.py
@@ -18,6 +18,7 @@
         self.down = ConvBN(cin, cout, 1, stride) if (stride != 1 or cin != cout) else None
 
     fused = True
+    _next = None
 
     def forward(self, x):
         if self.fused and resnet_fused.fused_ok(self, x):
@@ -26,6 +27,12 @@
         y = self.c1(x)
         y = self.c2(y)
         return self.c3(y, residual=idn, relu=True)
+
+
+def chain_blocks(blocks):
+    blocks = list(blocks)
+    for a, b in zip(blocks, blocks[1:]):
+        a._next = (b,)
 
 
 class ResNet(nn.Module):
@@ -39,6 +46,7 @@
             for j in range(n):
                 blocks.append(Bottleneck(cin, w, stride=2 if (j == 0 and i > 0) else 1))
                 cin = w * Bottleneck.expansion
+        chain_blocks(blocks)
         self.blocks = nn.Sequential(*blocks)
         self.fc = Linear(cin, num_classes, init_std=0.01)
 
diff --git a/distributed-tensorflow-guide_amd/models/resnet_fused.py b/distributed-tensorflow-guide_amd/models/resnet_fused.py
--- a/distributed-tensorflow-guide_amd/models/resnet_fused.py
+++ b/distributed-tensorflow-guide_amd/models/resnet_fused.py
@@ -34,6 +34,51 @@
 _DXD2 = True
 _DXD_S2 = True
 _dxd_calls = 0
+_FWD1 = True
+_FWD1_S2 = True
+_fwd1_calls = 0
+
+
+class _Conv1Ahead:
+    __slots__ = ("out", "w_ptr", "w_ver", "y1n", "part")
+
+    def __init__(self, out, w, wm, y1n, part):
+        self.out, self.w_ptr, self.w_ver, self.y1n, self.part = out, wm.data_ptr(), w._version, y1n, part
+
+    def matches(self, x2, w, wm):
+        return (self.part is not None and x2.data_ptr() == self.out.data_ptr() and x2.shape == self.out.shape
+                and wm.data_ptr() == self.w_ptr and w._version == self.w_ver and wm.shape[0] == self.y1n.shape[1])
+
+    def take(self):
+        r = (self.y1n, self.part)
+        self.out = self.y1n = self.part = None
+        return r
+
+    def drop(self):
+        if self.part is not None:
+            self.part.zero_()
+        self.out = self.y1n = self.part = None
+
+    def __del__(self):
+        try:
+            self.drop()
+        except Exception:
+            pass
+
+
+def _next_conv1(blk, x, rows, cout):
+    nxt = getattr(blk, "_next", None)
+    nxt = nxt[0] if nxt else None
+    if nxt is None or not nxt.fused or not _fused_ok(nxt, x.is_cuda, x.dtype, cout):
+        return None
+    w = nxt.c1.conv.weight
+    if w.shape[1] != cout or w.device != x.device:
+        return None
+    if not lib().bn_apply_gemm_ok(rows, cout, w.shape[0]) or (cout == 512 and not _FWD1_S2):
+        return None
+    if blk.down is not None and cout == 256 and w.shape[0] != 64:
+        return None
+    return w
 
 
 class _Bn3Link:
@@ -79,7 +124,8 @@
 
 class _BottleneckFn(torch.autograd.Function):
     @staticmethod
-    def forward(ctx, x, blk, link_in, holder, *params):
+    def forward(ctx, x, blk, link_in, holder, ahead, *params):
+        global _fwd1_calls
         L = lib()
         n, c, h, w = x.shape
         st = blk.c2.conv.stride
@@ -89,8 +135,15 @@
         p_, q_ = (h + 2 - 3) // st + 1, (w + 2 - 3) // st + 1
         b1, b2, b3 = blk.c1.bn, blk.c2.bn, blk.c3.bn
         w1, w2, w3 = blk.c1.conv.weight, blk.c2.conv.weight, blk.c3.conv.weight
+        if ahead is not None and not (_FUSE and ahead.matches(x2, w1, _mat(w1))):
+            ahead.drop()
+            ahead = None
         if _FUSE:
-            y1, p1 = L.gemm_bn(x2, _mat(w1), 1, pooled=True)
+            if ahead is not None:
+                y1, p1 = ahead.take()
+                _fwd1_calls += 1
+            else:
+                y1, p1 = L.gemm_bn(x2, _mat(w1), 1, pooled=True)
             bits1 = _relu_bits(y1)
             a1, m1, i1 = L.bn_fwd_part(y1, p1, None, b1.weight, b1.bias, b1.running_mean, b1.running_var,
                                        b1.momentum, b1.eps, True, bits=bits1)
@@ -131,14 +184,22 @@
         bits = None
         if _FUSE and _LINK:
             bits = torch.empty(y3.shape[0], cout // 8, device=y3.device, dtype=torch.uint8)
+        wn = _next_conv1(blk, x, y3.shape[0], cout) if (_FUSE and _FWD1) else None
+        nkw, y1n = {}, None
+        if wn is not None:
+            nkw = dict(next_w=_mat(wn.detach()), next_part=L.bn_part_alloc(y3, wn.shape[0], pooled=True))
         if _FUSE and blk.down is not None:
             assert bd.momentum == b3.momentum and bd.eps == b3.eps
-            out, m3, i3, md, idd = L.bn_fwd2_part(y3, p3, b3.weight, b3.bias, b3.running_mean, b3.running_var, yd, pd,
-                                                  bd.weight, bd.bias, bd.running_mean, bd.running_var, b3.momentum,
-                                                  b3.eps, bits=bits)
+            r = L.bn_fwd2_part(y3, p3, b3.weight, b3.bias, b3.running_mean, b3.running_var, yd, pd,
+                               bd.weight, bd.bias, bd.running_mean, bd.running_var, b3.momentum,
+                               b3.eps, bits=bits, **nkw)
+            out, m3, i3, md, idd = r[:5]
+            y1n = r[5] if nkw else None
         elif _FUSE:
-            out, m3, i3 = L.bn_fwd_part(y3, p3, idn, b3.weight, b3.bias, b3.running_mean, b3.running_var,
-                                        b3.momentum, b3.eps, True, bits=bits)
+            r = L.bn_fwd_part(y3, p3, idn, b3.weight, b3.bias, b3.running_mean, b3.running_var,
+                              b3.momentum, b3.eps, True, bits=bits, **nkw)
+            out, m3, i3 = r[:3]
+            y1n = r[3] if nkw else None
         else:
             out, m3, i3 = L.bn_fwd_train(y3, idn, b3.weight, b3.bias, b3.running_mean, b3.running_var, b3.momentum,
                                          b3.eps, True)
@@ -146,6 +207,7 @@
         ctx.link_in = link_in if (_FUSE and _LINK) else None
         ctx.link_out = _Bn3Link(y3, m3, i3, b3.weight, b3.bias, bits, yd, md, idd) if (_FUSE and _LINK) else None
         holder.append(ctx.link_out)
+        holder.append(_Conv1Ahead(out, wn, nkw["next_w"], y1n, nkw["next_part"]) if y1n is not None else None)
         ctx.geom = (n, c, h, w, st, width, cout, p_, q_)
         ctx.save_for_backward(x2, y1, a1, m1, i1, y2, a2, m2, i2, y3, out, m3, i3,
                               *((yd, md, idd) if yd is not None else ()))
@@ -307,13 +369,17 @@
                 grads.append(None)
             else:
                 grads.append(a.to(p.dtype))
-        return (dx2.view(n, h, w, c).permute(0, 3, 1, 2), None, None, None, *grads)
+        return (dx2.view(n, h, w, c).permute(0, 3, 1, 2), None, None, None, None, *grads)
+
+
+def _fused_ok(blk, is_cuda, dtype, cin):
+    ws = [blk.c1.conv.weight, blk.c2.conv.weight, blk.c3.conv.weight]
+    return (blk.training and is_cuda and dtype == torch.bfloat16 and all(v.dtype == torch.bfloat16 for v in ws)
+            and cin % 64 == 0 and blk.c1.conv.weight.shape[0] % 64 == 0)
 
 
 def fused_ok(blk, x):
-    ws = [blk.c1.conv.weight, blk.c2.conv.weight, blk.c3.conv.weight]
-    return (blk.training and x.is_cuda and x.dtype == torch.bfloat16 and all(v.dtype == torch.bfloat16 for v in ws)
-            and x.shape[1] % 64 == 0 and blk.c1.conv.weight.shape[0] % 64 == 0)
+    return _fused_ok(blk, x.is_cuda, x.dtype, x.shape[1])
 
 
 def bottleneck(blk, x):
@@ -322,9 +388,11 @@
     if blk.down is not None:
         params += [blk.down.conv.weight, blk.down.bn.weight, blk.down.bn.bias]
     holder = []
-    y = _BottleneckFn.apply(x, blk, getattr(x, "_dtg_bn3", None), holder, *params)
+    y = _BottleneckFn.apply(x, blk, getattr(x, "_dtg_bn3", None), holder, getattr(x, "_dtg_conv1", None), *params)
     if holder and holder[0] is not None:
         y._dtg_bn3 = holder[0]
+    if len(holder) > 1 and holder[1] is not None:
+        y._dtg_conv1 = holder[1]
     return y
 
 
```

Result: faster. 17760 images/sec (median of 6 runs) (+2.3%).
